# zilliztech/knowhere

Hardware: AMD Instinct MI355X
Metric: QPS at recall@10>=0.95, IVF-PQ 100M x d=128 batch=10k (higher is better)
Workload: dtype f32

## Files before the change

knowhere_amd/csrc/kernels.h:

```cpp
#pragma once

#include <hip/hip_runtime.h>
#include <stdint.h>
#include <algorithm>
#include "sq_codec.h"

namespace knhip {

struct KnItem {
    int32_t list;
    int32_t npair;
    int64_t pair0;
};
struct KnPair {
    int32_t q;
    int32_t slot;
};

__host__ __device__ constexpr int pq_stream_phase(int lane) {
    const int l = lane & 31;
    return l < 4 ? l : l < 12 ? l + 4 : l < 16 ? l - 8 : l < 20 ? l - 16 : l < 28 ? l - 12 : l - 24;
}
constexpr int PQ_STREAM_PHASES = 16;
__host__ __device__ constexpr uint32_t pq_stream_mask(int j) {
// ... 117 lines not shown
    const int64_t* list_sblk_off;
    const int64_t* list_len;
    const int64_t* list_row_off;
    const int64_t* ids;
    const float* precomp_t;
    const float* cb;
    const float* centroids;
    int32_t d;
    int32_t lut_mode;
    const float* queries;
    const float* t2t;
    const float* coarse_dis;
    const KnItem* items;
    const KnPair* pairs;
    const int64_t* nitems_dev;
    const uint8_t* bitset;
    int64_t bitset_nbits;
    float* partial_d;
    int64_t* partial_i;
    float* gthr;
    int32_t nslot;
    int32_t k;
    const int64_t* item_lo;
    const int64_t* item_hi;
    float* dump;
    int64_t dump_stride;
    int32_t dump_by_row;
    const int64_t* dump_pair_col;
    uint32_t* ghist;
    const uint2* gmeta;
    P4Rec* recs4;
    int32_t* q4_ctr;
    const float4* cb_t;
};


struct SqScanArgs {
    const uint4* rows;
    const int64_t* list_blk_off;
    const int64_t* list_len;
    const int64_t* list_row_off;
    const int64_t* ids;
    const float* trained;
    const float* centroids;
    int32_t d;
    int32_t nchunk16;
    int32_t bits;
    const float* queries;
    const float* coarse_dis;
    const KnItem* items;
    const KnPair* pairs;
    const int64_t* nitems_dev;
    const uint8_t* bitset;
    int64_t bitset_nbits;
    float* partial_d;
    int64_t* partial_i;
    float* gthr;
    int32_t nslot;
    int32_t k;
    float* dump;
    int64_t dump_stride;
    const int64_t* dump_pair_col;
    int32_t item_loop;
};

struct MScanArgs {
    const void* rows;
    const float* xnorm;
    float xnorm_max;
    const int64_t* list_blk_off;
    const int64_t* list_len;
    const int64_t* list_row_off;
    const int64_t* ids;
    const float* trained;
    const float* centroids;
    int32_t d;
    int32_t nchunk;
    int32_t nstep;
    int32_t sq_bits;
    int32_t row_type;
    const float* queries;
    const float* qnorm;
    const float* coarse_dis;
    int64_t nq;
    int32_t nslot;
    const KnItem* units;
    const KnPair* pairs;
    const int64_t* nunits_dev;
    const float* gthr;
    float eps_scale;
    const uint8_t* bitset;
    int64_t bitset_nbits;
    int32_t* cand_cnt;
    int64_t* cand;
    uint32_t* eps_max;
    float* cand_pess;
    int32_t cap;
    int32_t* overflow;
    float* dump;
    int64_t dump_stride;
    int32_t sample_cap;
    uint32_t* ghist;
    const uint2* gmeta;
    int32_t k;
    const int32_t* sample_off;
    const void* qh;
    const void* ql;
    const float* qs;
    int32_t unit_loop;
    float* gthr_rw;
    const uint4* pq_codes_r;
    const int64_t* pq_sblk_off_r;
    const float* pq_psum;
    const void* pq_qh;
    const float* pq_qs;
    const float4* pq_cb_t;
    const float* pq_precomp_t;
    const uint8_t* pq_codes;
    int32_t pq_lut_mode;
    P8Rec* pq_recs;
    const uint4* pq_codes_i;
    const void* pq_qi;
    const float* pq_qis;
    P16Rec* pq_recs16;
    int32_t* pq_ctr;
    int32_t pq_prune_mu;
    const void* pq_cb16;
    const void* pq_qh16;
    const float* pq_qd;
    const float* pq_sc;
    const float* pq_psum_s;
    unsigned char* pq_spill;
    int32_t pq_spill_cap;
    int32_t pq_spill_wgs;
    const int2* pq_unit_tiles;
};

int64_t pq_stream16r_blocks(int64_t len);
hipError_t launch_pq_stream16r(const uint8_t* codes, const int64_t* list_row_off, const int64_t* list_len,
                               const int64_t* list_sblk_off, int64_t nlist, uint4* out, hipStream_t s);
hipError_t launch_pq_psum(const uint8_t* codes, const int64_t* list_row_off, const int64_t* list_len,
                          const int64_t* list_sblk_off, int64_t nlist, const float* precomp_t, float* psum,
                          uint32_t* pabs_max_bits, hipStream_t s);
hipError_t launch_pqf_query_table(const float* queries, const float4* cb_m, int d, int64_t nq, bool is_l2, float pabs_max,
                                  void* qh, float* qs, hipStream_t s);
hipError_t launch_pqf_predict(const float* dump, int64_t stride, const int32_t* n_row, const float* gthr, const float* qs,
                              const float* qs2, const int64_t* keys, int nprobe, int64_t nlist, const int64_t* list_len,
                              int64_t nq, int cap, int k, bool is_l2, int32_t* poor, hipStream_t s);
size_t pqf_smem();
hipError_t launch_pq_stream16i(const uint8_t* codes, const int64_t* list_row_off, const int64_t* list_len,
                               const int64_t* list_sblk_off, int64_t nlist, uint4* out, hipStream_t s);
hipError_t launch_pqi_query_table(const float* queries, const float4* cb_m, int d, int64_t nq, bool is_l2, float pabs_max,
                                  void* qi, float* qis, float* qmu, bool stats_done, hipStream_t s);
hipError_t launch_pq_sample(const MScanArgs& a, const int64_t* keys, const float4* cb_m, int64_t nlist, int smin,
                            int scap, float pabs_max, bool is_l2, int32_t* n_row, float* qs, float* qis, float* qmu,
                            hipStream_t s, float* gthr_out = nullptr, uint2* gmeta_out = nullptr, int ksel = 0);
hipError_t launch_pqi(const MScanArgs& a, bool is_l2, int64_t units_bound, hipStream_t s);

constexpr int PD_QT = 128;
size_t pqd_smem();
bool pqd_supports(int M, int d);
hipError_t launch_pqd_index_prep(const float4* cb, const float* centroids, int64_t ncent, void* cb16, float* st,
                                 uint32_t* scratch, const float* psum, int64_t npsum, float* psum_s, hipStream_t s);
hipError_t launch_pqd_query_prep(const float* queries, const float4* cb, const float* cst, int64_t nq, bool is_l2,
                                 float pabs_max, void* qh16, float* qd, hipStream_t s);
hipError_t launch_pqd(const MScanArgs& a, bool is_l2, int64_t units_bound, hipStream_t s);

bool pqf_supports(int M, int d);
hipError_t launch_pqf(const MScanArgs& a, bool is_l2, int64_t units_bound, hipStream_t s);

int flat_scan_qg(int k);
int sq_scan_qg(int k);
hipError_t launch_flat_scan(const FlatScanArgs& a, bool is_l2, bool dense, int64_t grid, hipStream_t s,
                            int qg_override = 0);
hipError_t launch_flat_full(const FlatScanArgs& a, bool is_l2, float* out, const int32_t* q_subset,
                            int64_t nq_subset, const int32_t* row_flags, hipStream_t s);
hipError_t launch_interleave_rows(const float* src, int64_t n, int d, float4* dst, int64_t dst_blk0,
                                  hipStream_t s);
hipError_t launch_rows_narrow_check(const float* x, int64_t n, int d, int row_type, uint16_t* out,
                                    unsigned long long* first_bad, hipStream_t s);
hipError_t launch_rows_widen(const uint16_t* x, int64_t n_values, int row_type, float* out, hipStream_t s);
hipError_t launch_interleave_lists16(const uint16_t* src, const int64_t* list_row_off, const int64_t* list_len,
                                     const int64_t* list_blk_off, int64_t nlist, int d, uint4* dst, hipStream_t s);
hipError_t launch_interleave_lists(const float* src, const int64_t* list_row_off,
                                   const int64_t* list_len, const int64_t* list_blk_off, int64_t nlist,
                                   int d, float4* dst, hipStream_t s);

int pq_scan_supported_m(int M);
int pq_scan_qg(int M);
int64_t pq_skew_blocks(int64_t len, int M);
hipError_t launch_pq_scan(const PqScanArgs& a, bool is_l2, int M, int64_t grid, hipStream_t s);
hipError_t launch_pq_query_table(const float* queries, const float* cb, int d, int M, int64_t nq,
                                 float* t2t, hipStream_t s);
hipError_t launch_pq_precomp_table(const float* centroids, const float* cb, int d, int M,
                                   int64_t nlist, float* pt, hipStream_t s);
hipError_t launch_pq_skew_codes(const uint8_t* codes, const int64_t* list_row_off,
                                const int64_t* list_len, const int64_t* list_sblk_off, int64_t nlist,
                                int M, uint4* out, hipStream_t s);

bool pq_scan_v2_supports(int M, int k);
int64_t pq_stream16_blocks(int64_t len);
hipError_t launch_pq_scan_v2(const PqScanArgs& a, bool is_l2, bool dump, int64_t grid, hipStream_t s);
hipError_t launch_rank0_select(const float* dump, int64_t dump_stride, const int64_t* keys, int nprobe,
                               const int64_t* list_len, const int64_t* list_row_off, const int64_t* ids,
                               int64_t nq, int k, bool is_l2, float* partial_d, int64_t* partial_i, float* gthr,
                               int64_t* tmp_keys, float* tmp_d, uint32_t* ghist, uint2* gmeta, hipStream_t s);
hipError_t launch_pq_stream16(const uint8_t* codes, const int64_t* list_row_off, const int64_t* list_len,
                              const int64_t* list_sblk_off, int64_t nlist, uint4* out, hipStream_t s);

bool pq_scan_q4_supports(int M, int d, int k);
hipError_t launch_pq_scan_q4(const PqScanArgs& a, bool is_l2, int64_t items_bound, hipStream_t s);
hipError_t launch_pq_cb_transpose(const float* cb, int M, int dsub, float4* cb_t, hipStream_t s);

int mscan_queries_per_unit(int kind, bool sample);
size_t mscan_flat_smem(int nstep);
size_t mscan_sq8_smem(int nstep, int bits = 8);
int mscan_finish_pmax(int cap, int k);
int mscan_sample_rows();
hipError_t launch_ms_block_norms(const float4* rows, int64_t total_blk, int nchunk, float* out, float* out_max,
                                 hipStream_t s, int row_type = KN_ROW_FP32);
hipError_t launch_ms_sq8_norms(const uint4* rows, int64_t total_blk, int nchunk16, int d, const float* trained,
                               float* out, float* out_max, hipStream_t s, int bits = 8);
hipError_t launch_ms_units(const int32_t* list_count_v, const int64_t* list_pair_off_v, int64_t nlist, int qt,
                           int64_t* unit_off, int64_t* nunits, KnItem* units, const int64_t* list_len,
                           int64_t code_size, double* unit_bytes, hipStream_t s, int cost_cap = 0,
                           int2* unit_tiles = nullptr);
inline int64_t ms_units_cost_bound(int64_t npairs, int qt, int64_t nlist, int64_t ntotal, int64_t max_len, int cost_cap) {
    const int64_t groups = npairs / qt + std::min<int64_t>(nlist, npairs) + 1;
    if (cost_cap <= 0) {
        return groups;
    }
    const int64_t max_ntile = std::max<int64_t>((max_len + 31) / 32, 1);
    const int64_t by_cost = groups + (2 * max_ntile * (npairs / 32 + groups) + cost_cap - 1) / cost_cap;
    const int64_t by_tiles = npairs / qt * max_ntile + ntotal / 32 + 2 * nlist + 1;
    return std::max<int64_t>(groups, std::min<int64_t>(by_cost, by_tiles));
}
hipError_t launch_mscan_flat(const MScanArgs& a, bool is_l2, int64_t units_bound, hipStream_t s);
int mscan_flat_bf16_qt(int nstep);
size_t mscan_flat_bf16_smem(int nstep);
hipError_t launch_mscan_flat_bf16(const MScanArgs& a, bool is_l2, int64_t units_bound, hipStream_t s);
hipError_t launch_mscan_sq8(const MScanArgs& a, bool is_l2, int64_t units_bound, hipStream_t s);
hipError_t launch_ms_sample_plan(const int64_t* keys, int64_t nq, int nprobe, int64_t nlist, const int64_t* list_len,
                                 int smin, int cap, int32_t* sample_off, int32_t* n_row, hipStream_t s);
hipError_t launch_ms_sq8_query_prep(const float* queries, int64_t nq, int d, int ldq, const float* trained, void* qh,
                                    void* ql, float* qs, hipStream_t s, int bits = 8);
hipError_t launch_ms_tau(const float* sel_d, int64_t nq, int k, bool is_l2, float* gthr, uint2* gmeta, hipStream_t s);
hipError_t launch_mscan_finish(const MScanArgs& a, int kind, bool is_l2, const int64_t* keys, const float* coarse_dis,
                               int nprobe, int k, float* out_d, int64_t* out_i, unsigned long long* counters, int pass,
                               hipStream_t s);
hipError_t launch_ms_flag_pairs(const int32_t* overflow, int want, const int64_t* keys, int64_t nq, int nprobe,
                                int64_t nlist, const int64_t* list_len, int k, KnItem* items, KnPair* pairs,
                                int64_t* nitems, int64_t* empty_mark, hipStream_t s);

hipError_t launch_sq_scan(const SqScanArgs& a, bool is_l2, int64_t grid, hipStream_t s, int qg_override = 0);
hipError_t launch_sq_interleave(const uint8_t* codes, const int64_t* list_row_off,
                                const int64_t* list_len, const int64_t* list_blk_off, int64_t nlist,
                                int64_t code_size, uint4* out, hipStream_t s);

struct WorkTable {
    int32_t* list_count;
    int64_t* list_pair_off;
    int64_t* list_item_off;
    int32_t* list_cursor;
    KnPair* pairs;
    KnItem* items;
    int64_t* nitems;
    double* scan_bytes;
    int64_t* empty_mark;
    int32_t k;
};
hipError_t launch_direct_items(const int64_t* keys, int64_t nq, int nprobe, int64_t nlist, const int64_t* list_len,
                               const WorkTable& wt, hipStream_t s);
hipError_t launch_build_worktable(const int64_t* keys, int64_t nq, int nprobe, int64_t nlist, int qg0, int qg1,
                                  const int64_t* list_len, int64_t code_size, const WorkTable& wt,
                                  hipStream_t s, int rank0_slot = 0, const int32_t* cls = nullptr);
hipError_t launch_fill_f32(float* p, int64_t n, float v, hipStream_t s);

struct RangeArgs {
    const float* dist;
    int64_t ncol;
    const int64_t* seg_col;
    const int64_t* seg_idpos;
    const int64_t* seg_len;
    const int64_t* ids;
    int64_t id_offset;
    const int64_t* order;
    int32_t nprobe;
    float radius;
    const uint8_t* bitset;
    int64_t bitset_nbits;
    const float* radius_q;
    int32_t inclusive;
};
hipError_t launch_tie_detect(const float* d, const int64_t* i, int64_t nq, int k, float* out_d, int64_t* out_i,
                             int32_t* flagged, int32_t* nflag, hipStream_t s);
hipError_t launch_tie_gather(const int32_t* flagged, int nflag, const float* q, int d, const int64_t* keys, const float* cdis,
                             int nprobe, float* q_out, int64_t* keys_out, float* cdis_out, const float* can_d, int k,
                             float* rad_out, hipStream_t s);
hipError_t launch_tie_sort_flags(const int32_t* in, int n, int32_t* out, hipStream_t s);
hipError_t launch_refine_combine(const float* parts, int nsh, int64_t n, float* out, hipStream_t s);
hipError_t launch_tie_resolve(const int32_t* flagged, int nflag, int nsh, const float* can_d, const int64_t* can_i, int k,
                              bool is_l2, const float* arr_d, const int64_t* arr_i, const int64_t* arr_key,
                              const int64_t* arr_n, int64_t arr_n_stride, float* out_d, int64_t* out_i, int32_t* anomalies,
                              hipStream_t s);
struct PqDumpArgs {
    float* dist;
    int64_t ncol;
    const int64_t* pair_col;
    const int64_t* keys;
    const float* coarse_dis;
    int32_t nprobe;
    int64_t nlist;
    const int64_t* list_len;
    const int64_t* list_row_off;
// ... 184 lines not shown
```

knowhere_amd/csrc/knhip_api.hip:

```cpp
#include "knhip_internal.h"

namespace knhip_host {

thread_local std::string g_last_error;

int fail(int code, const std::string& msg) {
    g_last_error = msg;
    return code;
}

int build_coarse_layout(knhip_index* idx) {
    const int nchunk = (idx->d + 3) / 4;
    const int64_t nblk = (idx->nlist + 63) / 64;
    HIP_TRY(idx->centroids_il.alloc((size_t)nblk * nchunk * 64 * sizeof(float4)));
    HIP_TRY(launch_interleave_rows(idx->centroids.as<float>(), idx->nlist, idx->d,
                                   idx->centroids_il.as<float4>(), 0, nullptr));
    HIP_TRY(idx->cnorm.alloc((size_t)idx->nlist * sizeof(float)));
    HIP_TRY(launch_row_norms(idx->centroids.as<float>(), idx->nlist, idx->d, idx->cnorm.as<float>(), nullptr));
    HIP_TRY(idx->centroids_bs.alloc((size_t)idx->nlist * coarse_bf16_slabs(idx->d) * 128));
    HIP_TRY(launch_coarse_bf16_split(idx->centroids.as<float>(), idx->nlist, idx->d, idx->centroids_bs.p, nullptr));
    HIP_TRY(hipDeviceSynchronize());
    std::vector<float> cn((size_t)idx->nlist);
    HIP_TRY(hipMemcpy(cn.data(), idx->cnorm.p, cn.size() * sizeof(float), hipMemcpyDeviceToHost));
    idx->cnorm_max = cn.empty() ? 0.f : *std::max_element(cn.begin(), cn.end());
// ... 255 lines not shown
    idx->h_list_blk_off = blk_off;
    if (kind == KNHIP_IVF_FLAT && idx->row_type != KNHIP_ROWTYPE_FP32) {
        const int nchunk = row_nchunk(idx->d, idx->row_type);
        HIP_TRY(idx->rows.alloc((size_t)total_blk * nchunk * 64 * sizeof(uint4)));
        HIP_TRY(launch_interleave_lists16(reinterpret_cast<const uint16_t*>(d_codes), idx->d_list_row_off.as<int64_t>(),
                                          idx->d_list_len.as<int64_t>(), idx->d_list_blk_off.as<int64_t>(), nlist, idx->d,
                                          idx->rows.as<uint4>(), nullptr));
    } else if (kind == KNHIP_IVF_FLAT) {
        const int nchunk = (idx->d + 3) / 4;
        HIP_TRY(idx->rows.alloc((size_t)total_blk * nchunk * 64 * sizeof(float4)));
        HIP_TRY(launch_interleave_lists(reinterpret_cast<const float*>(d_codes),
                                        idx->d_list_row_off.as<int64_t>(), idx->d_list_len.as<int64_t>(),
                                        idx->d_list_blk_off.as<int64_t>(), nlist, idx->d,
                                        idx->rows.as<float4>(), nullptr));
    } else if (kind == KNHIP_IVF_PQ) {
        const int M = idx->desc.pq_m;
        idx->pq_v2 = (M == 32) && !idx->pq_v1;
        idx->rows.release();
        idx->skew_ready = false;
        if (!idx->pq_v2 && pq_scan_supported_m(M)) {
            if (int rc2 = build_pq_skew(idx)) return rc2;
        }
        if (idx->pq_v2) {
            std::vector<int64_t> off2(nlist + 1, 0);
            for (int64_t l = 0; l < nlist; l++) {
                off2[l + 1] = off2[l] + pq_stream16_blocks(idx->h_list_len[l]);
            }
            if ((rc = upload(idx->d_list_blk_off2, off2.data(), (nlist + 1) * sizeof(int64_t)))) return rc;
            HIP_TRY(idx->rows2.alloc((size_t)off2[nlist] * 64 * sizeof(uint4)));
            HIP_TRY(launch_pq_stream16(d_codes, idx->d_list_row_off.as<int64_t>(), idx->d_list_len.as<int64_t>(),
                                       idx->d_list_blk_off2.as<int64_t>(), nlist, idx->rows2.as<uint4>(), nullptr));
        }
    } else if (kind == KNHIP_IVF_SQ8) {
        const int nchunk16 = sq_nchunk16(idx->d, idx->sq_bits);
        HIP_TRY(idx->rows.alloc((size_t)total_blk * nchunk16 * 64 * sizeof(uint4)));
        HIP_TRY(launch_sq_interleave(d_codes, idx->d_list_row_off.as<int64_t>(),
                                     idx->d_list_len.as<int64_t>(), idx->d_list_blk_off.as<int64_t>(),
                                     nlist, idx->code_size, idx->rows.as<uint4>(), nullptr));
    } else {
        return fail(KNHIP_ERR_INVALID_ARGS, "lists on a brute-force index");
    }
    HIP_TRY(hipDeviceSynchronize());
    if (!keep_aos) {
        idx->codes_aos.release();
    }
    idx->has_data = true;
    return KNHIP_OK;
}

int ensure_aos(const knhip_index* cidx) {
    knhip_index* idx = const_cast<knhip_index*>(cidx);
    if (idx->aos_ready || !idx->has_data || idx->desc.kind == KNHIP_BRUTE_FORCE) {
        return KNHIP_OK;
    }
    HIP_TRY(idx->codes_aos.alloc((size_t)std::max<int64_t>(idx->ntotal, 1) * idx->dev_code_size()));
    HIP_TRY(launch_deinterleave_lists(idx->rows.as<uint4>(), idx->d_list_row_off.as<int64_t>(),
                                      idx->d_list_len.as<int64_t>(), idx->d_list_blk_off.as<int64_t>(), idx->nlist,
                                      idx->dev_code_size(), idx->codes_aos.as<uint8_t>(), nullptr));
    HIP_TRY(hipDeviceSynchronize());
    idx->aos_ready = true;
    return KNHIP_OK;
}

int ensure_mscan_norms(const knhip_index* idx) {
    const int64_t total_blk = idx->total_blk;
    std::lock_guard<std::mutex> lk(idx->mu);
    if (idx->xnorm_ready) {
        return KNHIP_OK;
    }
    HIP_TRY(idx->xnorm.alloc((size_t)std::max<int64_t>(total_blk, 1) * 64 * sizeof(float) + 16));
    float* xn = idx->xnorm.as<float>();
    float* xmax = xn + std::max<int64_t>(total_blk, 1) * 64;
    if (idx->desc.kind == KNHIP_IVF_FLAT) {
        HIP_TRY(launch_ms_block_norms(idx->rows.as<float4>(), total_blk, row_nchunk(idx->d, idx->row_type), xn, xmax, nullptr,
                                      idx->row_type));
        HIP_TRY(hipDeviceSynchronize());
        HIP_TRY(hipMemcpy(&idx->xnorm_max, xmax, sizeof(float), hipMemcpyDeviceToHost));
    } else {
        HIP_TRY(launch_ms_sq8_norms(idx->rows.as<uint4>(), total_blk, sq_nchunk16(idx->d, idx->sq_bits), idx->d,
                                    idx->sq_trained.as<float>(), xn, xmax, nullptr, idx->sq_bits));
        HIP_TRY(hipDeviceSynchronize());
        HIP_TRY(hipMemcpy(&idx->xnorm_max, xmax, sizeof(float), hipMemcpyDeviceToHost));
    }
    idx->xnorm_ready = true;
    return KNHIP_OK;
}

int ensure_psum(const knhip_index* idx) {
    std::lock_guard<std::mutex> lk(idx->mu);
    if (idx->psum_ready) {
        return KNHIP_OK;
    }
    const int64_t nlist = idx->nlist;
    std::vector<int64_t> off(nlist + 1, 0);
    for (int64_t l = 0; l < nlist; l++) {
        off[l + 1] = off[l] + pq_stream16r_blocks(idx->h_list_len[l]);
    }
    HIP_TRY(idx->d_list_blk_off_r.alloc((size_t)(nlist + 1) * sizeof(int64_t)));
    HIP_TRY(hipMemcpy(idx->d_list_blk_off_r.p, off.data(), (size_t)(nlist + 1) * sizeof(int64_t), hipMemcpyHostToDevice));
    idx->pabs_max = 0.f;
    if (idx->is_l2) {
        const size_t npos = (size_t)std::max<int64_t>(off[nlist], 1) * 16;
        HIP_TRY(idx->psum.alloc((npos + 4) * sizeof(float)));
        HIP_TRY(hipMemset(idx->psum.p, 0, (npos + 4) * sizeof(float)));
        uint32_t* bits = reinterpret_cast<uint32_t*>(idx->psum.as<float>() + npos);
        HIP_TRY(launch_pq_psum(idx->codes_aos.as<uint8_t>(), idx->d_list_row_off.as<int64_t>(),
                               idx->d_list_len.as<int64_t>(), idx->d_list_blk_off_r.as<int64_t>(), nlist,
                               idx->precomp_t.as<float>(), idx->psum.as<float>(), bits, nullptr));
        HIP_TRY(hipDeviceSynchronize());
        HIP_TRY(hipMemcpy(&idx->pabs_max, bits, sizeof(float), hipMemcpyDeviceToHost));
    }
    HIP_TRY(hipDeviceSynchronize());
    idx->psum_ready = true;
    return KNHIP_OK;
}

int ensure_pqf(const knhip_index* idx) {
    if (int rc = ensure_psum(idx)) return rc;
    std::lock_guard<std::mutex> lk(idx->mu);
    if (idx->pqf_ready) {
        return KNHIP_OK;
    }
    const int64_t nblk = idx->nlist > 0 ? [&] {
        int64_t t = 0;
        for (int64_t l = 0; l < idx->nlist; l++) t += pq_stream16r_blocks(idx->h_list_len[l]);
        return t;
    }() : 0;
    HIP_TRY(idx->rows_r.alloc((size_t)std::max<int64_t>(nblk, 1) * 64 * sizeof(uint4)));
    HIP_TRY(launch_pq_stream16r(idx->codes_aos.as<uint8_t>(), idx->d_list_row_off.as<int64_t>(),
                                idx->d_list_len.as<int64_t>(), idx->d_list_blk_off_r.as<int64_t>(), idx->nlist,
                                idx->rows_r.as<uint4>(), nullptr));
    HIP_TRY(hipDeviceSynchronize());
    idx->pqf_ready = true;
    return KNHIP_OK;
}

int ensure_pqd(const knhip_index* idx) {
    if (int rc = ensure_psum(idx)) return rc;
    std::lock_guard<std::mutex> lk(idx->mu);
    if (idx->pqd_ready) {
        return KNHIP_OK;
    }
    HIP_TRY(idx->pqd_cb16.alloc((size_t)32 * 256 * 4 * 2));
    HIP_TRY(idx->pqd_st.alloc(16 * sizeof(float)));
    const int64_t npsum = idx->is_l2 ? (int64_t)(idx->psum.bytes / sizeof(float)) - 4 : 0;
    if (npsum > 0) {
        HIP_TRY(idx->psum_s.alloc((size_t)(npsum + 64) * sizeof(float)));
        HIP_TRY(hipMemset(idx->psum_s.p, 0, (size_t)(npsum + 64) * sizeof(float)));
    }
    HIP_TRY(launch_pqd_index_prep(idx->cb.as<float4>(), idx->centroids.as<float>(), idx->nlist * (int64_t)idx->d,
                                  idx->pqd_cb16.p, idx->pqd_st.as<float>(),
                                  reinterpret_cast<uint32_t*>(idx->pqd_st.as<float>() + 8), idx->psum.as<float>(), npsum,
                                  idx->psum_s.as<float>(), nullptr));
    HIP_TRY(hipDeviceSynchronize());
    idx->pqd_ready = true;
    return KNHIP_OK;
}

int ensure_pqi(const knhip_index* idx) {
    if (int rc = ensure_pqf(idx)) return rc;
    std::lock_guard<std::mutex> lk(idx->mu);
    if (idx->pqi_ready) {
        return KNHIP_OK;
    }
    const int64_t nblk = idx->rows_r.bytes / (64 * sizeof(uint4));
    HIP_TRY(idx->rows_i.alloc((size_t)std::max<int64_t>(nblk, 1) * 64 * sizeof(uint4)));
    HIP_TRY(launch_pq_stream16i(idx->codes_aos.as<uint8_t>(), idx->d_list_row_off.as<int64_t>(),
                                idx->d_list_len.as<int64_t>(), idx->d_list_blk_off_r.as<int64_t>(), idx->nlist,
                                idx->rows_i.as<uint4>(), nullptr));
    HIP_TRY(hipDeviceSynchronize());
    idx->pqi_ready = true;
    return KNHIP_OK;
}

Workspace* acquire_ws(const knhip_index* idx, void* stream_key, bool pooled_by_stream) {
    std::lock_guard<std::mutex> lk(idx->mu);
    if (pooled_by_stream) {
        auto& slot = idx->ws_by_stream[stream_key];
        if (!slot) {
            slot.reset(new Workspace());
        }
        return slot.get();
    }
    if (!idx->ws_free.empty()) {
        Workspace* w = idx->ws_free.back().release();
        idx->ws_free.pop_back();
        return w;
    }
    return new Workspace();
}

void release_ws(const knhip_index* idx, Workspace* w) {
    std::lock_guard<std::mutex> lk(idx->mu);
    idx->ws_free.emplace_back(w);
}

int ensure_bf_split(const knhip_index* idx) {
    std::lock_guard<std::mutex> lk(idx->mu);
    if (idx->bf_split_ready) {
        return KNHIP_OK;
    }
    const int64_t nb = idx->ntotal;
    const int nslab = coarse_bf16_slabs(idx->d);
    HIP_TRY(idx->rows_bs.alloc((size_t)std::max<int64_t>(nb, 1) * nslab * 128));
    HIP_TRY(idx->bf_norm.alloc((size_t)std::max<int64_t>(nb, 1) * sizeof(float)));
    HIP_TRY(launch_coarse_bf16_split(idx->codes_aos.as<float>(), nb, idx->d, idx->rows_bs.p, nullptr));
    HIP_TRY(launch_row_norms(idx->codes_aos.as<float>(), nb, idx->d, idx->bf_norm.as<float>(), nullptr));
    HIP_TRY(hipDeviceSynchronize());
    std::vector<float> h((size_t)nb);
    HIP_TRY(hipMemcpy(h.data(), idx->bf_norm.p, h.size() * sizeof(float), hipMemcpyDeviceToHost));
    float mx = 0.f;
    for (float v : h) {
        mx = v > mx ? v : mx;
    }
    idx->bf_norm_max = mx;
    idx->bf_split_ready = true;
    return KNHIP_OK;
}

void note_route(const knhip_index* idx, bool bf_mfma, int pq_form, bool rank0_phase, int64_t items_bound) {
    std::lock_guard<std::mutex> lk(idx->mu);
    idx->last_bf_mfma = bf_mfma ? 1 : 0;
    idx->last_pq_form = pq_form;
    idx->rank0_phase_used = rank0_phase;
    idx->last_items_bound = items_bound;
}

}

extern "C" {

int knhip_device_memory(int32_t device, int64_t* free_bytes, int64_t* total_bytes) {
    int n = 0;
    if (hipGetDeviceCount(&n) != hipSuccess || device < 0 || device >= n) {
        return fail(KNHIP_ERR_INVALID_ARGS, "device_memory: no such device");
    }
    DeviceGuard g(device);
    size_t f = 0, t = 0;
    HIP_TRY(hipMemGetInfo(&f, &t));
    if (free_bytes) *free_bytes = (int64_t)f;
    if (total_bytes) *total_bytes = (int64_t)t;
    return KNHIP_OK;
}

int knhip_abi_version(void) {
    return KNHIP_ABI_VERSION;
}

int knhip_device_count(void) {
    int n = 0;
    if (hipGetDeviceCount(&n) != hipSuccess) {
        return 0;
    }
    return n;
}

const char* knhip_last_error(void) {
    return g_last_error.c_str();
}

int knhip_index_create(const knhip_desc* desc, knhip_index** out) {
    if (!desc || !out) {
        return fail(KNHIP_ERR_INVALID_ARGS, "null argument");
    }
    *out = nullptr;
    if (desc->kind < KNHIP_BRUTE_FORCE || desc->kind > KNHIP_IVF_SQ8) {
        return fail(KNHIP_ERR_INVALID_ARGS, "unknown index kind");
    }
    if (desc->metric != KNHIP_L2 && desc->metric != KNHIP_IP) {
        return fail(KNHIP_ERR_INVALID_ARGS, "metric must be L2 or IP (cosine is normalised IP)");
    }
    if (desc->dim <= 0 || desc->dim > 32768) {
        return fail(KNHIP_ERR_INVALID_ARGS, "dim out of range");
    }
    if (desc->kind != KNHIP_BRUTE_FORCE && (desc->nlist <= 0 || desc->nlist > (1 << 24))) {
        return fail(KNHIP_ERR_INVALID_ARGS, "nlist out of range");
    }
    if (desc->kind == KNHIP_IVF_PQ) {
        if (desc->pq_nbits < 1 || desc->pq_nbits > 8) {
            return fail(KNHIP_ERR_NOT_IMPLEMENTED, "PQ codes of 1 .. 8 bits are supported");
        }
        if (desc->pq_m <= 0 || desc->dim % desc->pq_m != 0) {
            return fail(KNHIP_ERR_INVALID_ARGS, "pq_m must divide dim");
        }
        if (!pq_scan_supported_m(desc->pq_m) && !pq_scan_any_supports(desc->pq_m, desc->dim)) {
            return fail(KNHIP_ERR_NOT_IMPLEMENTED, "pq_m above 128, or sub-vectors of more than 144 dimensions");
        }
    }
    int ndev = knhip_device_count();
    if (ndev <= 0) {
        return fail(KNHIP_ERR_HIP_RUNTIME, "no HIP device visible");
    }
    if (desc->device < 0 || desc->device >= ndev) {
        return fail(KNHIP_ERR_INVALID_ARGS, "device ordinal out of range");
    }
    std::unique_ptr<knhip_index> idx(new knhip_index());
    idx->desc = *desc;
    idx->is_l2 = desc->metric == KNHIP_L2;
    idx->d = desc->dim;
    idx->nlist = desc->kind == KNHIP_BRUTE_FORCE ? 0 : desc->nlist;
    switch (desc->kind) {
        case KNHIP_BRUTE_FORCE:
        case KNHIP_IVF_FLAT:
            idx->code_size = (int64_t)desc->dim * 4;
            break;
        case KNHIP_IVF_PQ:
// ... 997 lines not shown
    }
    return KNHIP_OK;
}

int knhip_index_get_sq(const knhip_index* idx, float* vmin, float* vdiff) {
    if (int rc = check_index(idx)) return rc;
    if (!idx->has_sq || !vmin || !vdiff) {
        return fail(KNHIP_ERR_NOT_TRAINED, "SQ parameters not set");
    }
    DeviceGuard g(idx->desc.device);
    HIP_TRY(hipMemcpy(vmin, idx->sq_trained.p, (size_t)idx->d * sizeof(float), hipMemcpyDeviceToHost));
    HIP_TRY(hipMemcpy(vdiff, idx->sq_trained.as<float>() + idx->d, (size_t)idx->d * sizeof(float), hipMemcpyDeviceToHost));
    return KNHIP_OK;
}

int knhip_index_get_list_sizes(const knhip_index* idx, int64_t* sizes) {
    if (int rc = check_index(idx)) return rc;
    if (idx->desc.kind == KNHIP_BRUTE_FORCE || !sizes) {
        return fail(KNHIP_ERR_INVALID_ARGS, "get_list_sizes: not an IVF index");
    }
    for (int64_t l = 0; l < idx->nlist; l++) {
        sizes[l] = idx->has_data ? idx->h_list_len[l] : 0;
    }
    return KNHIP_OK;
}

int knhip_index_get_lists(const knhip_index* idx, uint8_t* codes, int64_t* ids) {
    if (int rc = check_index(idx)) return rc;
    if (!idx->has_data) {
        return KNHIP_OK;
    }
    DeviceGuard g(idx->desc.device);
    std::lock_guard<std::mutex> add_lk(const_cast<knhip_index*>(idx)->add_mu);
    if (codes) {
        if (int rc = ensure_aos(idx)) return rc;
        const size_t b = idx->desc.kind == KNHIP_BRUTE_FORCE ? (size_t)idx->ntotal * idx->d * sizeof(float)
                                                             : (size_t)idx->ntotal * idx->code_size;
        if (idx->desc.kind == KNHIP_IVF_PQ && idx->desc.pq_nbits != 8) {
            const int nb_pq = idx->desc.pq_nbits, M = idx->desc.pq_m;
            const size_t cs_out = ((size_t)M * nb_pq + 7) / 8;
            std::vector<uint8_t> h(b);
            HIP_TRY(hipMemcpy(h.data(), idx->codes_aos.p, b, hipMemcpyDeviceToHost));
            std::memset(codes, 0, (size_t)idx->ntotal * cs_out);
            for (int64_t i = 0; i < idx->ntotal; i++) {
                uint8_t* dst = codes + (size_t)i * cs_out;
                const uint8_t* src = h.data() + (size_t)i * M;
                for (int m = 0; m < M; m++) {
                    const size_t bit = (size_t)m * nb_pq;
                    const uint32_t v = (uint32_t)src[m] << (bit & 7);
                    dst[bit >> 3] |= (uint8_t)v;
                    if ((bit & 7) + (size_t)nb_pq > 8) {
                        dst[(bit >> 3) + 1] |= (uint8_t)(v >> 8);
                    }
                }
            }
        } else if (idx->row_type != KNHIP_ROWTYPE_FP32) {
            DevBuf wide;
            HIP_TRY(wide.alloc(b));
            HIP_TRY(launch_rows_widen(idx->codes_aos.as<uint16_t>(), idx->ntotal * idx->d, idx->row_type, wide.as<float>(), nullptr));
            HIP_TRY(hipMemcpy(codes, wide.p, b, hipMemcpyDeviceToHost));
        } else {
            HIP_TRY(hipMemcpy(codes, idx->codes_aos.p, b, hipMemcpyDeviceToHost));
        }
    }
    if (ids && idx->desc.kind != KNHIP_BRUTE_FORCE) {
        HIP_TRY(hipMemcpy(ids, idx->ids.p, (size_t)idx->ntotal * sizeof(int64_t), hipMemcpyDeviceToHost));
    }
    return KNHIP_OK;
}

int knhip_index_get_vectors_device(const knhip_index* idx, const float** d_rows) {
    if (int rc = check_index(idx)) return rc;
    if (idx->desc.kind != KNHIP_BRUTE_FORCE || !d_rows) {
        return fail(KNHIP_ERR_INVALID_ARGS, "get_vectors_device: brute-force index only");
    }
    *d_rows = idx->codes_aos.as<float>();
    return KNHIP_OK;
}

int knhip_profile_enable(knhip_index* idx, int on) {
    if (int rc = check_index(idx)) return rc;
    idx->prof = on != 0;
    return KNHIP_OK;
}

static void drain_pending(const knhip_index* idx) {
    std::vector<PendingEvent> p;
    {
        std::lock_guard<std::mutex> lk(idx->mu);
        p.swap(idx->pending);
    }
    for (auto& e : p) {
        float ms = 0.f;
        if (hipEventSynchronize(e.e1) == hipSuccess && hipEventElapsedTime(&ms, e.e0, e.e1) == hipSuccess) {
            idx->times.ms[e.stage] += ms;
            idx->times.launches[e.stage] += 1;
        }
        (void)hipEventDestroy(e.e0);
        (void)hipEventDestroy(e.e1);
    }
}

int knhip_profile_reset(knhip_index* idx) {
    if (int rc = check_index(idx)) return rc;
    DeviceGuard g(idx->desc.device);
    drain_pending(idx);
    std::memset(&idx->times, 0, sizeof(idx->times));
    idx->coarse_flops = 0;
    idx->tie_queries = 0;
    HIP_TRY(hipDeviceSynchronize());
    HIP_TRY(hipMemset(idx->scan_bytes_dev.p, 0, 3 * sizeof(double)));
    HIP_TRY(hipMemset(idx->coarse_fail_dev.p, 0, 8 * sizeof(unsigned long long)));
    return KNHIP_OK;
}

int knhip_profile_get(const knhip_index* idx, knhip_stage_times* out) {
    if (int rc = check_index(idx)) return rc;
    if (!out) {
        return fail(KNHIP_ERR_INVALID_ARGS, "null output");
    }
    DeviceGuard g(idx->desc.device);
    HIP_TRY(hipDeviceSynchronize());
    drain_pending(idx);
    double sb[3] = {0, 0, 0};
    HIP_TRY(hipMemcpy(sb, idx->scan_bytes_dev.p, 3 * sizeof(double), hipMemcpyDeviceToHost));
    *out = idx->times;
    out->scan_bytes = sb[0];
    out->scan_bytes_rank0 = idx->rank0_phase_used ? sb[1] : 0.0;
    out->coarse_flops = idx->coarse_flops;
    out->tie_queries = idx->tie_queries;
    out->scan_items = idx->last_items_bound;
    unsigned long long nf[6] = {0, 0, 0, 0, 0, 0};
    HIP_TRY(hipMemcpy(nf, idx->coarse_fail_dev.p, sizeof(nf), hipMemcpyDeviceToHost));
    out->tie_anomalies = (int64_t)(nf[5] & 0xffffffffull);
    out->coarse_fallback_queries = (int64_t)nf[0];
    out->mscan_queries = (int64_t)nf[1];
    out->mscan_overflow_queries = (int64_t)nf[2];
    out->mscan_candidates = (int64_t)nf[3];
    out->mscan_recomputed = (int64_t)nf[4];
    out->pq_filter_form = idx->desc.kind == KNHIP_BRUTE_FORCE ? (idx->last_bf_mfma ? 10 : 0) : idx->last_pq_form;
    out->mscan_stream_bytes = sb[2];
    return KNHIP_OK;
}

const char* knhip_stage_kernel_name(int stage, int kind) {
    switch (stage) {
        case KNHIP_STAGE_COARSE:
            return "coarse_bf16_kernel (two passes)+coarse_bound_kernel+coarse_rerank_kernel | coarse_gemm_kernel+row_select_thr_kernel";
        case KNHIP_STAGE_GROUP:
            return "wt_*_kernel+ms_unit*_kernel";
        case KNHIP_STAGE_LUT:
            return "pq_query_table_kernel";
        case KNHIP_STAGE_SCAN_RANK0:
            return kind == KNHIP_IVF_PQ ? "pq_sample_kernel | pq_scan_v2_kernel<DUMP>+row_select_kernel"
                                        : "mscan_flat_kernel<DUMP> | mscan_sq8_kernel<DUMP> +row_select_kernel+ms_tau_kernel";
        case KNHIP_STAGE_TABLES:
            return "pqi_query_table_kernel | pqf_query_table_kernel +pqf_predict_kernel";
        case KNHIP_STAGE_SCAN:
            return kind == KNHIP_IVF_PQ    ? "pqi_kernel | pqf_kernel | pq_scan_q4_kernel | pq_scan_kernel | pq_scan_any_kernel"
                   : kind == KNHIP_IVF_SQ8 ? "mscan_sq8_kernel | sq_scan_kernel"
                                           : "mscan_flatb_kernel | mscan_flat_kernel | flat_scan_kernel";
        case KNHIP_STAGE_MERGE:
            return "mscan_finish_kernel | merge_partials_kernel";
        case KNHIP_STAGE_REFINE:
            return "refine_kernel";
        case KNHIP_STAGE_TIES:
            return "tie_detect_kernel+range dump pass+tie_resolve_kernel";
        default:
            return "other";
    }
}

}
```

knowhere_amd/csrc/knhip_api_search.hip:

```cpp
#include "knhip_internal.h"

namespace knhip_host {

template <class A>
static A scan_args(const knhip_index* idx, const Workspace* ws, const Batch& b) {
    A a{};
    a.list_len = idx->d_list_len.as<int64_t>();
    a.list_row_off = idx->d_list_row_off.as<int64_t>();
    a.ids = idx->ids.as<int64_t>();
    a.d = idx->d;
    a.queries = b.q;
    a.bitset = b.bitset;
    a.bitset_nbits = b.nbits;
    a.partial_d = ws->partial_d.as<float>();
    a.partial_i = ws->partial_i.as<int64_t>();
    a.k = b.k;
    return a;
}
template <class A>
static A item_scan_args(const knhip_index* idx, const Workspace* ws, const Batch& b, const WorkTable& wt) {
    A a = scan_args<A>(idx, ws, b);
    a.items = wt.items;
    a.pairs = wt.pairs;
    a.nitems_dev = wt.nitems;
// ... 338 lines not shown
    a.item_hi = wt.nitems;
    if (plan.pq_rank0) {
        const int64_t stride = round_up(std::max<int64_t>(idx->max_list_len, 64), 64);
        HIP_TRY(ws->dump.reserve((size_t)b.nq * stride * sizeof(float)));
        HIP_TRY(ws->sel_keys.reserve((size_t)b.nq * b.k * sizeof(int64_t)));
        HIP_TRY(ws->sel_d.reserve((size_t)b.nq * b.k * sizeof(float)));
        HIP_TRY(ws->ghist.reserve((size_t)b.nq * 64 * sizeof(uint32_t)));
        HIP_TRY(ws->gmeta.reserve((size_t)b.nq * sizeof(uint2)));
        a.dump = ws->dump.as<float>();
        a.dump_stride = stride;
        a.item_lo = nullptr;
        a.item_hi = wt.list_item_off + nlist;
        const int64_t boundA = round_up(b.nq / plan.qg_rank0 + std::min<int64_t>(nlist, b.nq) + 1, 8);
        {
            StageTimer t(idx, s, KNHIP_STAGE_SCAN_RANK0);
            HIP_TRY(launch_pq_scan_v2(a, is_l2, true, boundA, s));
            HIP_TRY(launch_rank0_select(a.dump, stride, b.keys, b.nprobe, idx->d_list_len.as<int64_t>(),
                                        idx->d_list_row_off.as<int64_t>(), idx->ids.as<int64_t>(), b.nq, b.k, is_l2, a.partial_d,
                                        a.partial_i, a.gthr, ws->sel_keys.as<int64_t>(), ws->sel_d.as<float>(),
                                        idx->cand_hist ? ws->ghist.as<uint32_t>() : nullptr, ws->gmeta.as<uint2>(), s));
        }
        if (idx->cand_hist) {
            a.ghist = ws->ghist.as<uint32_t>();
            a.gmeta = ws->gmeta.as<uint2>();
        }
        a.item_lo = wt.list_item_off + nlist;
        a.item_hi = wt.nitems;
    }
    StageTimer t(idx, s, KNHIP_STAGE_SCAN);
    if (plan.pq_q4) {
        if (int rc = pq_q4_bind(idx, ws, plan.items_bound, &a)) return rc;
        HIP_TRY(launch_pq_scan_q4(a, is_l2, plan.items_bound, s));
    } else {
        HIP_TRY(launch_pq_scan_v2(a, is_l2, false, plan.items_bound, s));
    }
    return KNHIP_OK;
}

hipError_t launch_filter(const knhip_index* idx, const SearchPlan& plan, const PqForm& f, const MScanArgs& x, int64_t bound,
                         hipStream_t s) {
    const int kind = idx->desc.kind;
    const bool is_l2 = idx->is_l2;
    return kind == KNHIP_IVF_FLAT ? ((plan.flat_bf16 && x.dump == nullptr) ? launch_mscan_flat_bf16(x, is_l2, bound, s)
                                                                            : launch_mscan_flat(x, is_l2, bound, s))
         : kind == KNHIP_IVF_SQ8  ? launch_mscan_sq8(x, is_l2, bound, s)
         : (f.form == 3 && x.dump == nullptr) ? launch_pqd(x, is_l2, bound, s)
         : (f.form == 2 && x.dump == nullptr) ? launch_pqi(x, is_l2, bound, s)
                                              : launch_pqf(x, is_l2, bound, s);
}

int ms_common_args(const knhip_index* idx, Workspace* ws, const SearchPlan& plan, const Batch& b, const WorkTable& wt,
                   hipStream_t s, MScanArgs& m) {
    const int kind = idx->desc.kind;
    const int64_t nq = b.nq, nlist = idx->nlist;
    if (kind == KNHIP_IVF_PQ) {
        if (int rc = ensure_psum(idx)) return rc;
    } else {
        if (int rc = ensure_mscan_norms(idx)) return rc;
    }
    const int64_t max_units = std::max(plan.ms_units_bound, plan.ms_bound0);
    HIP_TRY(ws->ms_units.reserve((size_t)max_units * sizeof(KnItem)));
    HIP_TRY(ws->ms_unit_off.reserve((size_t)(nlist + 1) * sizeof(int64_t)));
    HIP_TRY(ws->ms_nunits.reserve(sizeof(int64_t) + 2 * sizeof(double)));
    HIP_TRY(ws->ms_cand.reserve((size_t)nq * plan.ms_cap * sizeof(int64_t)));
    HIP_TRY(ws->ms_cand_pess.reserve((size_t)nq * plan.ms_cap * sizeof(float)));
    if (kind == KNHIP_IVF_SQ8) {
        HIP_TRY(ws->ms_eps_max.reserve((size_t)nq * sizeof(uint32_t)));
        HIP_TRY(hipMemsetAsync(ws->ms_eps_max.p, 0, (size_t)nq * sizeof(uint32_t), s));
    }
    HIP_TRY(ws->ms_cand_cnt.reserve((size_t)(2 * nq + 4) * sizeof(int32_t)));
    HIP_TRY(ws->dump.reserve((size_t)nq * mscan_sample_rows() * sizeof(float)));
    HIP_TRY(ws->sel_keys.reserve((size_t)nq * b.k * sizeof(int64_t)));
    HIP_TRY(ws->sel_d.reserve((size_t)nq * b.k * sizeof(float)));
    HIP_TRY(ws->ghist.reserve((size_t)nq * 64 * sizeof(uint32_t)));
    HIP_TRY(ws->gmeta.reserve((size_t)nq * sizeof(uint2)));
    m = MScanArgs{};
    m.rows = idx->rows.p;
    m.xnorm = idx->xnorm.as<float>();
    m.xnorm_max = idx->xnorm_max;
    m.list_blk_off = idx->d_list_blk_off.as<int64_t>();
    m.list_len = idx->d_list_len.as<int64_t>();
    m.list_row_off = idx->d_list_row_off.as<int64_t>();
    m.ids = idx->ids.as<int64_t>();
    m.trained = idx->sq_trained.as<float>();
    m.centroids = idx->centroids.as<float>();
    m.d = idx->d;
    m.nchunk = plan.ms_nchunk;
    m.nstep = plan.ms_nstep;
    m.sq_bits = kind == KNHIP_IVF_SQ8 ? idx->sq_bits : 0;
    m.row_type = idx->row_type;
    m.queries = b.q;
    m.qnorm = ws->qnorm.as<float>();
    m.coarse_dis = b.cdis;
    m.nq = nq;
    m.nslot = b.nprobe;
    m.units = ws->ms_units.as<KnItem>();
    m.pairs = wt.pairs;
    m.nunits_dev = ws->ms_nunits.as<int64_t>();
    m.gthr = ws->gthr.as<float>();
    m.eps_scale = plan.ms_eps_fp32 + (plan.flat_bf16 ? 6.103515625e-5f : 0.f);
    m.bitset = b.bitset;
    m.bitset_nbits = b.nbits;
    m.cand_cnt = ws->ms_cand_cnt.as<int32_t>();
    m.cand = ws->ms_cand.as<int64_t>();
    m.cand_pess = ws->ms_cand_pess.as<float>();
    m.eps_max = kind == KNHIP_IVF_SQ8 ? ws->ms_eps_max.as<uint32_t>() : nullptr;
    m.cap = plan.ms_cap;
    m.overflow = m.cand_cnt + nq;
    m.gthr_rw = ws->gthr.as<float>();
    m.k = b.k;
    if (idx->cand_hist) {
        m.ghist = ws->ghist.as<uint32_t>();
        m.gmeta = ws->gmeta.as<uint2>();
    }
    if (kind == KNHIP_IVF_PQ) {
        HIP_TRY(ws->pq_recs.reserve((size_t)std::max<int64_t>(max_units, plan.npairs) * sizeof(P8Rec)));
        HIP_TRY(ws->pq_ctr.reserve(8 * 16 * sizeof(int32_t)));
        m.list_blk_off = nullptr;
        m.pq_sblk_off_r = idx->d_list_blk_off_r.as<int64_t>();
        m.pq_psum = idx->psum.as<float>();
        m.pq_cb_t = idx->cb_t.as<float4>();
        m.pq_precomp_t = idx->precomp_t.as<float>();
        m.pq_codes = idx->codes_aos.as<uint8_t>();
        m.pq_lut_mode = plan.lut_mode;
        m.pq_recs = ws->pq_recs.as<P8Rec>();
        m.pq_ctr = ws->pq_ctr.as<int32_t>();
    }
    return KNHIP_OK;
}

int ms_fork_group(const knhip_index* idx, Workspace* ws, const SearchPlan& plan, const Batch& b, const EnvSearch& env,
                  const WorkTable& wt, hipStream_t s, SideJoin* sj, WorkTable* wside) {
    *wside = wt;
    if (!plan.wt1_lazy) {
        if (!env.no_side_stream) {
            HIP_TRY(ws->wt[1].reserve(idx->nlist, plan.npairs, plan.items_bound));
            *wside = ws->wt[1].bind(nullptr, wt.empty_mark, wt.k);
        }
        wside->scan_bytes = reinterpret_cast<double*>(ws->ms_nunits.as<int64_t>() + 1);
    }
    if (env.no_side_stream) {
        return KNHIP_OK;
    }
    if (int rc = ensure_side_stream(ws)) return rc;
    HIP_TRY(hipEventRecord(ws->ev_fork, s));
    HIP_TRY(hipStreamWaitEvent(ws->side, ws->ev_fork, 0));
    HIP_TRY(launch_build_worktable(b.keys, b.nq, b.nprobe, idx->nlist, plan.qg, plan.qg, idx->d_list_len.as<int64_t>(),
                                   idx->dev_code_size(), *wside, ws->side, -1));
    HIP_TRY(hipEventRecord(ws->ev_join, ws->side));
    sj->forked = true;
    return KNHIP_OK;
}

int ms_sample_pass(const knhip_index* idx, Workspace* ws, const SearchPlan& plan, const Batch& b, const EnvSearch& env,
                   const WorkTable& wt, hipStream_t s, MScanArgs& m) {
    const int kind = idx->desc.kind, d = idx->d, k = b.k;
    const bool is_l2 = idx->is_l2;
    const int64_t nq = b.nq, nlist = idx->nlist, sample = mscan_sample_rows();
    StageTimer t(idx, s, KNHIP_STAGE_SCAN_RANK0);
    HIP_TRY(hipMemsetAsync(m.cand_cnt, 0, (size_t)(2 * nq + 1) * sizeof(int32_t), s));
    if (kind == KNHIP_IVF_PQ) {
        HIP_TRY(ws->ms_qs.reserve((size_t)nq * 4 * sizeof(float)));
        HIP_TRY(ws->ms_nrow.reserve((size_t)nq * sizeof(int32_t)));
        m.pq_qs = ws->ms_qs.as<float>();
        if (plan.pq_want_i8) {
            HIP_TRY(ws->ms_qi.reserve((size_t)nq * 256 * 32));
            HIP_TRY(ws->ms_qis.reserve(((size_t)nq * 4 + 4) * sizeof(float)));
            HIP_TRY(ws->ms_qmu.reserve((size_t)nq * 32 * sizeof(float)));
        }
    } else if (kind == KNHIP_IVF_FLAT) {
        HIP_TRY(ws->qnorm.reserve((size_t)nq * sizeof(float)));
        m.qnorm = ws->qnorm.as<float>();
        HIP_TRY(launch_row_norms(b.q, nq, d, ws->qnorm.as<float>(), s));
    } else if (!is_l2) {
        const int ldq = plan.ms_nstep * (idx->sq_bits == 8 ? 32 : 64);
        HIP_TRY(ws->ms_qh.reserve((size_t)nq * ldq * 2));
        HIP_TRY(ws->ms_ql.reserve((size_t)nq * ldq * 2));
        HIP_TRY(ws->ms_qs.reserve((size_t)nq * 8 * sizeof(float)));
        HIP_TRY(launch_ms_sq8_query_prep(b.q, nq, d, ldq, idx->sq_trained.as<float>(), ws->ms_qh.p, ws->ms_ql.p,
                                         ws->ms_qs.as<float>(), s, idx->sq_bits));
        m.qh = ws->ms_qh.p;
        m.ql = ws->ms_ql.p;
        m.qs = ws->ms_qs.as<float>();
    }
    HIP_TRY(hipMemsetAsync(ws->ghist.p, 0, (size_t)nq * 64 * sizeof(uint32_t), s));
    MScanArgs ds = m;
    ds.eps_scale = plan.ms_eps_fp32;
    ds.dump = ws->dump.as<float>();
    ds.dump_stride = sample;
    ds.sample_cap = plan.ms_sample_cap;
    ds.ghist = nullptr;
    if (kind == KNHIP_IVF_PQ) {
        int scap = (int)sample;
        if (env.pq_sample_rows > 0) {
            scap = std::max(64, std::min((int)sample, env.pq_sample_rows));
        }
        const bool i8 = plan.pq_want_i8;
        HIP_TRY(launch_pq_sample(ds, b.keys, idx->cb.as<float4>(), nlist, std::max(1024, 8 * k), scap, idx->pabs_max, is_l2,
                                 ws->ms_nrow.as<int32_t>(), ws->ms_qs.as<float>(), i8 ? ws->ms_qis.as<float>() : nullptr,
                                 i8 ? ws->ms_qmu.as<float>() : nullptr, s, ws->gthr.as<float>(), ws->gmeta.as<uint2>(), k));
        return KNHIP_OK;
    }
    HIP_TRY(launch_ms_units(wt.list_count, wt.list_pair_off, nlist, plan.ms_qt0, ws->ms_unit_off.as<int64_t>(),
                            ws->ms_nunits.as<int64_t>(), ws->ms_units.as<KnItem>(), idx->d_list_len.as<int64_t>(), idx->dev_code_size(),
                            nullptr, s));
    ds.sample_off = ws->ms_sample_off.as<int32_t>();
    HIP_TRY(launch_filter(idx, plan, PqForm{}, ds, plan.ms_bound0, s));
    HIP_TRY(launch_row_select_var(ws->dump.as<float>(), sample, b.keys, b.nprobe, idx->d_list_len.as<int64_t>(), nq, k, is_l2,
                                  ws->sel_keys.as<int64_t>(), ws->sel_d.as<float>(), s, sample, ws->ms_nrow.as<int32_t>()));
    HIP_TRY(launch_ms_tau(ws->sel_d.as<float>(), nq, k, is_l2, ws->gthr.as<float>(), ws->gmeta.as<uint2>(), s));
    return KNHIP_OK;
}

int pq_bind_form(const knhip_index* idx, Workspace* ws, const SearchPlan& plan, const Batch& b, const EnvSearch& env, hipStream_t s,
                 MScanArgs& m, PqForm* f) {
    const int64_t nq = b.nq;
    if (f->form == 1) {
        if (int rc = ensure_pqf(idx)) return rc;
        m.pq_codes_r = idx->rows_r.as<uint4>();
        HIP_TRY(ws->ms_qh.reserve((size_t)nq * 256 * 32 * 2));
        HIP_TRY(launch_pqf_query_table(b.q, idx->cb.as<float4>(), idx->d, nq, idx->is_l2, idx->pabs_max, ws->ms_qh.p,
                                       ws->ms_qs.as<float>(), s));
        m.pq_qh = ws->ms_qh.p;
    }
    if (f->form == 2) {
        if (int rc = ensure_pqi(idx)) return rc;
        f->qt = 16;
        HIP_TRY(ws->pq_recs16.reserve((size_t)std::max<int64_t>(std::max(plan.ms_units_bound, plan.ms_bound0), plan.npairs) *
                                      sizeof(P16Rec)));
        m.pq_codes_r = idx->rows_r.as<uint4>();
        m.pq_codes_i = idx->rows_i.as<uint4>();
        m.pq_qi = ws->ms_qi.p;
        m.pq_qis = ws->ms_qis.as<float>();
        m.pq_recs16 = ws->pq_recs16.as<P16Rec>();
    }
    if (f->form == 3) {
        f->qt = PD_QT;
        if (env.pqd_unit_cost > 0) {
            f->pqd_cost = env.pqd_unit_cost;
            f->pqd_bound = round_up(ms_units_cost_bound(plan.npairs, PD_QT, idx->nlist, idx->ntotal, idx->max_list_len,
                                                        f->pqd_cost), 8);
            HIP_TRY(ws->ms_units.reserve((size_t)f->pqd_bound * sizeof(KnItem)));
            HIP_TRY(ws->pqd_tiles.reserve((size_t)f->pqd_bound * sizeof(int2)));
            m.units = ws->ms_units.as<KnItem>();
            m.pq_unit_tiles = ws->pqd_tiles.as<int2>();
        }
        m.pq_cb16 = idx->pqd_cb16.p;
        m.pq_qh16 = ws->ms_qh16.p;
        m.pq_qd = ws->ms_qd.as<float>();
        m.pq_sc = idx->pqd_st.as<float>();
        m.pq_psum_s = idx->psum_s.as<float>();
        m.pq_spill_cap = 4 * 8192;
        if (idx->pqd_spill_cap > 0) {
            m.pq_spill_cap = idx->pqd_spill_cap;
        }
        m.pq_spill_wgs = 512;
        int dev = 0, ncu = 0;
        (void)hipGetDevice(&dev);
        if (hipDeviceGetAttribute(&ncu, hipDeviceAttributeMultiprocessorCount, dev) == hipSuccess && ncu > 0) {
            m.pq_spill_wgs = ncu;
        }
        HIP_TRY(ws->pq_spill.reserve((size_t)m.pq_spill_wgs * m.pq_spill_cap * 80));
        m.pq_spill = static_cast<unsigned char*>(ws->pq_spill.p);
    }
    return KNHIP_OK;
}

int pq_choose_form(const knhip_index* idx, Workspace* ws, const SearchPlan& plan, const Batch& b, const EnvSearch& env,
                   hipStream_t s, MScanArgs& m, PqForm* f) {
    const int64_t nq = b.nq, sample = mscan_sample_rows();
    const int k = b.k, nprobe = b.nprobe;
    const bool is_l2 = idx->is_l2;
    const bool want_dec = pqd_supports(idx->desc.pq_m, idx->d) && (idx->pqf_form == 0 || idx->pqf_form == 3);
    if (plan.pq_want_i8) {
        HIP_TRY(launch_pqi_query_table(b.q, idx->cb.as<float4>(), idx->d, nq, is_l2, idx->pabs_max, ws->ms_qi.p,
                                       ws->ms_qis.as<float>(), ws->ms_qmu.as<float>(), true, s));
    }
    if (want_dec) {
        if (int rc = ensure_pqd(idx)) return rc;
        HIP_TRY(ws->ms_qh16.reserve((size_t)nq * 128 * 2));
        HIP_TRY(ws->ms_qd.reserve((size_t)nq * 4 * sizeof(float)));
        HIP_TRY(launch_pqd_query_prep(b.q, idx->cb.as<float4>(), idx->pqd_st.as<float>(), nq, is_l2, idx->pabs_max,
                                      ws->ms_qh16.p, ws->ms_qd.as<float>(), s));
    }
    const bool want2 = plan.pq_want_i8 || want_dec;
    const int form2 = want_dec ? 3 : 2;
    const float* qs2 = want_dec ? ws->ms_qd.as<float>() : plan.pq_want_i8 ? ws->ms_qis.as<float>() : nullptr;
    auto decide = [&](const int32_t* poor_h, int64_t n) -> int {
        if (want2 && (idx->pqf_form == form2 || (int64_t)poor_h[1] * 4 <= n)) {
            return form2;
        }
        return (int64_t)poor_h[0] * 4 > n ? 0 : 1;
    };
    int form = want2 ? form2 : 1;
    if (idx->pqf_guard) {
        int32_t* poor = ws->ms_cand_cnt.as<int32_t>() + 2 * nq + 1;
        bool predicted = false;
        auto predict = [&]() -> hipError_t {
            if (predicted) {
                return hipSuccess;
            }
            predicted = true;
            return launch_pqf_predict(ws->dump.as<float>(), sample, ws->ms_nrow.as<int32_t>(), ws->gthr.as<float>(),
                                      ws->ms_qs.as<float>(), qs2, b.keys, nprobe, idx->nlist, idx->d_list_len.as<int64_t>(), nq,
                                      plan.ms_cap, k, is_l2, poor, s);
        };
        bool sync_now = true;
        std::unique_lock<std::mutex> lk(idx->mu);
        const bool cached = idx->guard_cache.size() < 64 || idx->guard_cache.count({k, nprobe}) != 0;
        if (cached) {
            knhip_index::GuardEntry& e = idx->guard_cache[{k, nprobe}];
            if (e.pending && hipEventQuery(e.ev) == hipSuccess) {
                e.pending = false;
                e.form = decide(e.h_poor, e.pending_nq);
            }
            e.age++;
            if (e.form > 0 && !env.guard_sync && (e.age & 63) != 0) {
                sync_now = false;
                form = e.form;
                if (!e.pending && (e.age & 3) == 0) {
                    HIP_TRY(predict());
                    if (e.h_poor == nullptr) {
                        HIP_TRY(hipHostMalloc(reinterpret_cast<void**>(&e.h_poor), 2 * sizeof(int32_t)));
                        HIP_TRY(hipEventCreateWithFlags(&e.ev, hipEventDisableTiming));
                    }
                    HIP_TRY(hipMemcpyAsync(e.h_poor, poor, 2 * sizeof(int32_t), hipMemcpyDeviceToHost, s));
                    HIP_TRY(hipEventRecord(e.ev, s));
                    e.pending = true;
                    e.pending_nq = nq;
                }
            }
        }
        lk.unlock();
        if (sync_now) {
            HIP_TRY(predict());
            int32_t h_poor[2] = {0, 0};
            HIP_TRY(hipMemcpyAsync(h_poor, poor, 2 * sizeof(int32_t), hipMemcpyDeviceToHost, s));
            HIP_TRY(hipStreamSynchronize(s));
            form = decide(h_poor, nq);
            if (cached) {
                lk.lock();
                knhip_index::GuardEntry& e = idx->guard_cache[{k, nprobe}];
                if (!e.pending) {
                    e.form = form;
                }
            }
        }
        if (form == 0) {
            return KNHIP_PQF_ABANDONED;
        }
    }
    f->form = form;
    return pq_bind_form(idx, ws, plan, b, env, s, m, f);
}

int ms_group_units(const knhip_index* idx, Workspace* ws, const SearchPlan& plan, const Batch& b, const PqForm& f,
                   const WorkTable& wside, SideJoin* sj, hipStream_t s, MScanArgs& m) {
    const int64_t nlist = idx->nlist;
    StageTimer t(idx, s, KNHIP_STAGE_GROUP);
    if (sj->forked) {
        if (int rc = sj->join()) return rc;
    } else {
        HIP_TRY(launch_build_worktable(b.keys, b.nq, b.nprobe, nlist, plan.qg, plan.qg, idx->d_list_len.as<int64_t>(),
                                       idx->dev_code_size(), wside, s, -1));
    }
    m.pairs = wside.pairs;
    HIP_TRY(launch_ms_units(wside.list_count + nlist, wside.list_pair_off + nlist, nlist, f.qt, ws->ms_unit_off.as<int64_t>(),
                            ws->ms_nunits.as<int64_t>(), ws->ms_units.as<KnItem>(), idx->d_list_len.as<int64_t>(), idx->dev_code_size(),
                            idx->scan_bytes_dev.as<double>() + 2, s, f.pqd_cost, ws->pqd_tiles.as<int2>()));
    return KNHIP_OK;
}

int rows_exact_scan(const knhip_index* idx, Workspace* ws, const Batch& b, const WorkTable& wt, int64_t grid, bool one_pair,
                    hipStream_t s) {
    if (idx->desc.kind == KNHIP_IVF_FLAT) {
        FlatScanArgs a = flat_scan_args(idx, ws, b, wt);
        a.item_loop = one_pair;
        HIP_TRY(launch_flat_scan(a, idx->is_l2, false, grid, s, one_pair));
    } else {
        SqScanArgs a = sq_scan_args(idx, ws, b, wt);
        a.item_loop = one_pair;
        HIP_TRY(launch_sq_scan(a, idx->is_l2, grid, s, one_pair));
    }
    return KNHIP_OK;
}

int exact_one_pair_items(const knhip_index* idx, Workspace* ws, const SearchPlan& plan, const Batch& b, const WorkTable& wt,
                         hipStream_t s) {
    if (idx->desc.kind != KNHIP_IVF_PQ) {
        return rows_exact_scan(idx, ws, b, wt, std::min<int64_t>(plan.npairs, 4096), true, s);
    }
    if (!plan.pq_q4_ok && !idx->skew_ready) {
        if (int rc = build_pq_skew(idx)) return rc;
    }
    PqScanArgs a = pq_scan_args(idx, ws, b, wt);
    a.item_lo = nullptr;
    a.item_hi = wt.nitems;
    if (plan.pq_q4_ok) {
        if (int rc = pq_q4_bind(idx, ws, plan.npairs, &a)) return rc;
        HIP_TRY(launch_pq_scan_q4(a, idx->is_l2, plan.npairs, s));
    } else {
        HIP_TRY(launch_pq_scan(a, idx->is_l2, idx->desc.pq_m, plan.npairs, s));
    }
    return KNHIP_OK;
}

int ms_finish(const knhip_index* idx, Workspace* ws, const SearchPlan& plan, const Batch& b, const PqForm& f, const WorkTable& wt,
              const MScanArgs& m, hipStream_t s) {
    const int kind = idx->desc.kind, k = b.k, nprobe = b.nprobe;
    const bool is_l2 = idx->is_l2;
    const int64_t nq = b.nq, nlist = idx->nlist;
    StageTimer t(idx, s, KNHIP_STAGE_MERGE);
    unsigned long long* counters = idx->coarse_fail_dev.as<unsigned long long>() + 1;
    MScanArgs mf = m;
    if (f.form == 2) {
        mf.pq_qs = m.pq_qis;
        mf.pq_prune_mu = 1;
    }
    if (f.form == 3) {
        mf.pq_qs = m.pq_qd;
    }
    HIP_TRY(launch_mscan_finish(mf, kind, is_l2, b.keys, b.cdis, nprobe, k, b.out_d, b.out_i, counters, 1, s));
    HIP_TRY(launch_ms_flag_pairs(m.overflow, 2, b.keys, nq, nprobe, nlist, idx->d_list_len.as<int64_t>(), k, wt.items, wt.pairs,
                                 wt.nitems, nullptr, s));
    MScanArgs r = m;
    r.pairs = wt.pairs;
    r.units = wt.items;
    r.nunits_dev = wt.nitems;
    r.unit_loop = 1;
    r.pq_unit_tiles = nullptr;
    r.ghist = nullptr;
    r.gmeta = nullptr;
    HIP_TRY(launch_filter(idx, plan, f, r, plan.npairs, s));
    HIP_TRY(launch_mscan_finish(mf, kind, is_l2, b.keys, b.cdis, nprobe, k, b.out_d, b.out_i, counters, 2, s));
    HIP_TRY(launch_ms_flag_pairs(m.overflow, 1, b.keys, nq, nprobe, nlist, idx->d_list_len.as<int64_t>(), k, wt.items, wt.pairs,
                                 wt.nitems, ws->partial_i.as<int64_t>(), s));
    if (int rc = exact_one_pair_items(idx, ws, plan, b, wt, s)) return rc;
    HIP_TRY(launch_merge_partials(ws->partial_d.as<float>(), ws->partial_i.as<int64_t>(), nq, nprobe, k, (int64_t)nprobe * k, k,
                                  is_l2, b.out_d, b.out_i, s, m.overflow));
    return KNHIP_OK;
}

int run_prefilter(const knhip_index* idx, Workspace* ws, const SearchPlan& plan, const Batch& b, const EnvSearch& env,
                  const WorkTable& wt, hipStream_t s, PqForm* f) {
    MScanArgs m;
    if (int rc = ms_common_args(idx, ws, plan, b, wt, s, m)) return rc;
    SideJoin sj{ws, s};
    WorkTable wside;
    if (int rc = ms_fork_group(idx, ws, plan, b, env, wt, s, &sj, &wside)) return rc;
    if (int rc = ms_sample_pass(idx, ws, plan, b, env, wt, s, m)) return rc;
    f->qt = plan.ms_qt;
    {
        StageTimer t(idx, s, KNHIP_STAGE_TABLES);
        if (idx->desc.kind == KNHIP_IVF_PQ) {
            if (int rc = pq_choose_form(idx, ws, plan, b, env, s, m, f)) return rc;
        }
    }
    if (int rc = ms_group_units(idx, ws, plan, b, *f, wside, &sj, s, m)) return rc;
    {
        StageTimer t(idx, s, KNHIP_STAGE_SCAN);
        HIP_TRY(launch_filter(idx, plan, *f, m, std::max(plan.ms_units_bound, f->pqd_bound), s));
    }
    return ms_finish(idx, ws, plan, b, *f, wt, m, s);
}

int ivf_route(const knhip_index* idx, Workspace* ws, const SearchPlan& plan, const Batch& b, const EnvSearch& env, hipStream_t s,
              PqForm* f) {
    const int kind = idx->desc.kind;
    const bool ms = plan.route == Route::Prefilter;
    HIP_TRY(ws->wt[0].reserve(idx->nlist, plan.npairs, ms ? std::max<int64_t>(plan.npairs, plan.items_bound) : plan.items_bound));
    HIP_TRY(ws->partial_d.reserve((size_t)plan.npairs * b.k * sizeof(float)));
    HIP_TRY(ws->partial_i.reserve((size_t)plan.npairs * b.k * sizeof(int64_t)));
    const WorkTable wt = ws->wt[0].bind(idx->scan_bytes_dev.as<double>(), ws->partial_i.as<int64_t>(), b.k);
    if (!plan.wt1_lazy) {
        if (int rc = build_worktable(idx, ws, plan, b, wt, s)) return rc;
    }
    if (kind == KNHIP_IVF_PQ && plan.lut_mode != PQ_LUT_RESIDUAL && !(plan.pq_q4 && !plan.pq_rank0)) {
        if (int rc = pq_lut_stage(idx, ws, b, s)) return rc;
    }
    if (ms) {
        const int rc_ms = run_prefilter(idx, ws, plan, b, env, wt, s, f);
        if (rc_ms != KNHIP_PQF_ABANDONED) {
            return rc_ms;
        }
        if (int rc = build_worktable(idx, ws, plan, b, wt, s)) return rc;
    }
    if (kind == KNHIP_IVF_PQ) {
        if (int rc = pq_exact_scan(idx, ws, plan, b, wt, s)) return rc;
    } else {
        StageTimer t(idx, s, KNHIP_STAGE_SCAN);
        if (int rc = rows_exact_scan(idx, ws, b, wt, plan.items_bound, false, s)) return rc;
    }
    return merge_stage(idx, ws, b, b.nprobe, s);
}

}

int search_batch(const knhip_index* idx, Workspace* ws, const float* d_q, int64_t nq, int k, int nprobe,
                 const uint8_t* d_bitset, int64_t nbits, int64_t* d_out_i, float* d_out_d,
                 hipStream_t s, const int64_t* pre_keys, const float* pre_cdis) {
    HIP_TRY(ws->gthr.reserve((size_t)nq * sizeof(float)));
    HIP_TRY(launch_fill_f32(ws->gthr.as<float>(), nq, idx->is_l2 ? FLT_MAX : -FLT_MAX, s));
    Batch b{d_q, nq, k, nprobe, d_bitset, nbits, d_out_i, d_out_d, pre_keys, pre_cdis};
    if (idx->desc.kind != KNHIP_BRUTE_FORCE && pre_keys == nullptr) {
        HIP_TRY(ws->keys.reserve((size_t)nq * nprobe * sizeof(int64_t)));
        HIP_TRY(ws->cdis.reserve((size_t)nq * nprobe * sizeof(float)));
        StageTimer t(idx, s, KNHIP_STAGE_COARSE);
        if (int rc = coarse_stage(idx, ws, d_q, nq, nprobe, ws->keys.as<int64_t>(), ws->cdis.as<float>(), s)) {
            return rc;
        }
        b.keys = ws->keys.as<int64_t>();
        b.cdis = ws->cdis.as<float>();
    }
    const EnvSearch env = env_search();
    const SearchPlan plan = plan_search(idx, nq, k, nprobe, d_bitset != nullptr, env);
    PqForm form;
    int rc = KNHIP_OK;
    switch (plan.route) {
        case Route::BfMfma:    rc = bf_mfma_batch(idx, ws, b, plan.bf_per, s); break;
        case Route::BfRows:    rc = bf_rows_batch(idx, ws, b, s); break;
        case Route::PqAny:     rc = pq_any_batch(idx, ws, plan, b, s); break;
        case Route::Exact:
        case Route::Prefilter: rc = ivf_route(idx, ws, plan, b, env, s, &form); break;
    }
    note_route(idx, plan.route == Route::BfMfma, form.form, plan.route == Route::Exact && plan.pq_v2 && plan.pq_rank0,
               plan.items_bound);
    return rc;
}

int validate_search(const knhip_index* idx, int64_t nq, int32_t k, int32_t& nprobe) {
    if (nq < 0 || k <= 0) {
        return fail(KNHIP_ERR_INVALID_ARGS, "nq must be >= 0 and k > 0");
    }
    if (k > KNHIP_MAX_K) {
        return fail(KNHIP_ERR_INVALID_ARGS, "k > 16384 is not supported");
    }
    const int kind = idx->desc.kind;
    if (kind == KNHIP_BRUTE_FORCE) {
        if (!idx->has_data) {
            return fail(KNHIP_ERR_EMPTY_INDEX, "brute-force index holds no vectors");
        }
        return KNHIP_OK;
    }
    if (!idx->has_coarse) {
        return fail(KNHIP_ERR_NOT_TRAINED, "coarse centroids not set");
    }
    if (kind == KNHIP_IVF_PQ && !idx->has_pq) {
        return fail(KNHIP_ERR_NOT_TRAINED, "PQ codebooks not set");
    }
    if (kind == KNHIP_IVF_SQ8 && !idx->has_sq) {
        return fail(KNHIP_ERR_NOT_TRAINED, "SQ parameters not set");
    }
    if (!idx->has_data) {
        return fail(KNHIP_ERR_EMPTY_INDEX, "inverted lists not set");
    }
    if (nprobe <= 0) {
        return fail(KNHIP_ERR_INVALID_ARGS, "nprobe must be > 0");
    }
    if (nprobe > idx->nlist) {
        nprobe = (int32_t)idx->nlist;
    }
    if ((size_t)nprobe > row_select_max_k()) {
        return fail(KNHIP_ERR_NOT_IMPLEMENTED, "nprobe > 65536 is not supported");
    }
    return KNHIP_OK;
}

int64_t query_batch(const knhip_index* idx, int64_t nq, int k, int nprobe) {
    double per_q;
    if (idx->desc.kind == KNHIP_BRUTE_FORCE) {
        const int64_t chunk_rows = bf_chunk_rows(idx->ntotal);
        const int64_t nchunks = (idx->ntotal + chunk_rows - 1) / chunk_rows;
        per_q = (double)nchunks * k * 12.0;
    } else {
        per_q = (double)idx->nlist * 4.0 + (double)nprobe * (12.0 + 8.0 + (double)k * 12.0);
        if ((size_t)nprobe > row_select_lds_max_k()) {
            per_q += 16.0 * nprobe;
        }
        if ((idx->desc.kind == KNHIP_IVF_FLAT || idx->desc.kind == KNHIP_IVF_SQ8) && idx->mscan != 0) {
            per_q += 4.0 * mscan_sample_rows() + 8.0 * 32768.0;
        }
        if (idx->desc.kind == KNHIP_IVF_PQ && idx->pqf != 0) {
            per_q += 4.0 * mscan_sample_rows() + 12.0 * 32768.0 + 16384.0 + 8192.0 + (double)nprobe * (256.0 + 96.0);
        }
        if (idx->desc.kind == KNHIP_IVF_PQ) {
            per_q += 256.0 * idx->desc.pq_m * 4.0;
            if (!pq_scan_supported_m(idx->desc.pq_m)) {
                per_q += (double)nprobe * (pq_scan_any_parts(k) - 1) * (double)k * 12.0;
            }
        }
    }
    const double budget = 8.0 * 1024 * 1024 * 1024;
    int64_t qb = (int64_t)(budget / std::max(per_q, 1.0));
    qb = std::max<int64_t>(qb, 8);
    qb = std::min<int64_t>(qb, 65536 * 16);
    return std::min(qb, std::max<int64_t>(nq, 1));
}

}
```

knowhere_amd/csrc/knhip_env.h:

```cpp
#pragma once
#include <algorithm>
#include <cstdlib>
#include <cstring>

namespace knhip_host {

struct EnvLayout {
    bool coarse_given;
    int coarse_gemm;
    size_t aos_keep_bytes;
    bool rank0_select;
    bool cand_hist;
    int pq_q4;
    int mscan;
    bool flat_bf16;
    int mscan_cap;
    int pqd_spill_cap;
    int pqf;
    bool pqf_guard;
    int pqf_form;
    bool pq_v1;
    bool bf_exact;
    int pq_waves;
};

struct EnvSearch {
    int ms_sample_rows;
    int pq_sample_rows;
    bool no_side_stream;
    bool guard_sync;
    bool range_no_waves;
    bool ties_canonical;
    bool ties_trace;
    int pqd_unit_cost;
    size_t largek_round_bytes;
};
constexpr int KNHIP_PQD_UNIT_COST_DEFAULT = 512;

inline bool env_is(const char* v, const char* what) { return v != nullptr && std::strcmp(v, what) == 0; }
inline int env_digit(const char* v, int lo, int hi, int dflt) { return (v && v[0] >= '0' + lo && v[0] <= '0' + hi) ? v[0] - '0' : dflt; }
inline int env_count(const char* v) { return (v && *v) ? std::max(0, std::atoi(v)) : 0; }

inline EnvLayout env_layout() {
    EnvLayout e{};
    const char* c = std::getenv("KNHIP_COARSE");
    e.coarse_given = c != nullptr;
    e.coarse_gemm = env_is(c, "exact") ? 0 : env_is(c, "fp32") ? 1 : 2;
    const char* keep = std::getenv("KNHIP_AOS_KEEP_MB");
    e.aos_keep_bytes = (keep && *keep) ? (size_t)std::max<long long>(0, std::atoll(keep)) << 20 : (size_t)8 << 30;
    const char* r0 = std::getenv("KNHIP_RANK0");
    e.rank0_select = !(r0 && r0[0] == '0');
    const char* h = std::getenv("KNHIP_HIST");
    e.cand_hist = !(h && h[0] == '0');
    e.pq_q4 = env_digit(std::getenv("KNHIP_Q4"), 0, 2, 2);
    e.mscan = env_digit(std::getenv("KNHIP_MSCAN"), 0, 2, 2);
    e.flat_bf16 = !env_is(std::getenv("KNHIP_MSCAN_FLAT"), "fp32");
    e.mscan_cap = env_count(std::getenv("KNHIP_MSCAN_CAP"));
    e.pqd_spill_cap = env_count(std::getenv("KNHIP_PQD_SPILL"));
    const char* pf = std::getenv("KNHIP_PQF");
    e.pqf = (pf && pf[0] == '1') ? 2 : (pf && pf[0] == '0') ? 0 : 1;
    const char* pg = std::getenv("KNHIP_PQF_GUARD");
    e.pqf_guard = !(pg && pg[0] == '0');
    const char* pm = std::getenv("KNHIP_PQF_FORM");
    e.pqf_form = (pm && pm[0] == 'h') ? 1 : (pm && pm[0] == 'i') ? 2 : (pm && pm[0] == 'd') ? 3 : 0;
    const char* v1 = std::getenv("KNHIP_PQ_V1");
    e.pq_v1 = v1 && v1[0] == '1';
    e.bf_exact = env_is(std::getenv("KNHIP_BF"), "exact");
    const char* w = std::getenv("KNHIP_PQ_WAVES");
    e.pq_waves = w ? std::atoi(w) : 8;
    return e;
}

inline long long env_add_slice_rows(int d) {
    const char* v = std::getenv("KNHIP_ADD_SLICE_ROWS");
    if (v && *v && std::atoll(v) > 0) {
        return std::atoll(v);
    }
    return std::max<long long>(1, ((long long)1 << 30) / ((long long)d * 4));
}

inline EnvSearch env_search() {
    EnvSearch e{};
    const char* a = std::getenv("KNHIP_MS_SAMPLE_ROWS");
    e.ms_sample_rows = a ? std::max(1, std::atoi(a)) : 0;
    const char* b = std::getenv("KNHIP_PQ_SAMPLE_ROWS");
    e.pq_sample_rows = b ? std::max(1, std::atoi(b)) : 0;
    e.no_side_stream = std::getenv("KNHIP_NO_SIDE_STREAM") != nullptr;
    e.guard_sync = std::getenv("KNHIP_PQF_GUARD_SYNC") != nullptr;
    e.range_no_waves = std::getenv("KNHIP_RANGE_NO_WAVES") != nullptr;
    const char* t = std::getenv("KNHIP_TIES");
    e.ties_canonical = t && (t[0] == 'c' || t[0] == 'C' || t[0] == '0');
    e.ties_trace = std::getenv("KNHIP_TIES_TRACE") != nullptr;
    const char* uc = std::getenv("KNHIP_PQD_UNIT_COST");
    e.pqd_unit_cost = (uc && *uc) ? std::max(0, std::atoi(uc)) : KNHIP_PQD_UNIT_COST_DEFAULT;
    const char* lk = std::getenv("KNHIP_LARGEK_ROUND_KB");
    e.largek_round_bytes = (lk && *lk) ? (size_t)std::max<long long>(1, std::atoll(lk)) << 10 : (size_t)2 << 30;
    return e;
}

}
```

knowhere_amd/csrc/knhip_internal.h:

```cpp
#pragma once
#include "../../include/knhip.h"
#include "common.h"
#include "kernels.h"
#include "knhip_env.h"

#include <cstdio>
#include <cstdlib>
#include <cstring>
#include <map>
#include <memory>
#include <mutex>
#include <numeric>
#include <random>
#include <string>
#include <vector>

using namespace knhip;

namespace knhip_host {

int fail(int code, const std::string& msg);

#define HIP_TRY(expr)                                                                              \
    do {                                                                                           \
// ... 78 lines not shown
                         empty_mark,               k};
    }
};

struct Workspace {
    DevBuf coarse_full;
    DevBuf keys;
    DevBuf cdis;
    DevBuf t2t;
    DevBuf partial_d;
    DevBuf partial_i;
    DevBuf gthr;
    DevBuf qnorm;
    DevBuf cand_keys;
    DevBuf cand_approx;
    DevBuf fail_flags;
    DevBuf dump;
    DevBuf sel_keys;
    DevBuf sel_d;
    DevBuf rg_seg, rg_cnt, rg_off, rg_tot, rg_out_i, rg_out_d;
    DevBuf cg_gmin, cg_bound, cg_cnt, cg_qs;
    DevBuf rg_state, rg_keys_w, rg_cdis_w;
    DevBuf recs4;
    DevBuf q4_ctr;
    DevBuf ghist;
    DevBuf gmeta;
    WorkTableBufs wt[2];
    DevBuf ms_qi, ms_qis, ms_qmu, pq_recs16;
    DevBuf rs_ovf;
    DevBuf ms_eps_max;
    DevBuf ms_cand_pess;
    DevBuf ms_units, ms_unit_off, ms_nunits, ms_cand, ms_cand_cnt;
    DevBuf ms_sample_off, ms_nrow;
    DevBuf ms_qh, ms_ql, ms_qs;
    DevBuf pq_recs, pq_ctr;
    DevBuf bf_kth;
    DevBuf ms_qh16, ms_qd, pq_spill;
    DevBuf pqd_tiles;
    DevBuf rs_sort;
    DevBuf h_queries, h_bitset, h_out_d, h_out_i, h_ref_d, h_ref_i;
    DevBuf tie_d, tie_i, tie_flag, tie_q, tie_r, tie_keys, tie_cdis;
    DevBuf tie_arr_d, tie_arr_i, tie_arr_n;
    DevBuf lk_plan, lk_scratch;
    std::mutex mu;
    hipStream_t side = nullptr;
    hipEvent_t ev_fork = nullptr, ev_join = nullptr;
    volatile int32_t* h_word = nullptr;
    int32_t word_seq = 0;
    ~Workspace() {
        if (h_word) (void)hipHostFree(const_cast<int32_t*>(h_word));
        if (ev_fork) (void)hipEventDestroy(ev_fork);
        if (ev_join) (void)hipEventDestroy(ev_join);
        if (side) (void)hipStreamDestroy(side);
    }
};

struct SideJoin {
    Workspace* ws;
    hipStream_t s;
    bool forked = false;
    int join() {
        if (forked) {
            forked = false;
            HIP_TRY(hipStreamWaitEvent(s, ws->ev_join, 0));
        }
        return 0;
    }
    ~SideJoin() {
        (void)join();
    }
};

struct PendingEvent {
    int stage;
    hipEvent_t e0, e1;
};

}
using namespace knhip_host;

struct knhip_index {
    knhip_desc desc{};
    bool is_l2 = true;
    int64_t nlist = 0;
    int d = 0;
    bool has_coarse = false;
    DevBuf centroids;
    DevBuf centroids_il;
    DevBuf cnorm;
    DevBuf centroids_bs;
    float cnorm_max = 0.f;
    int coarse_gemm = 2;
    DevBuf coarse_fail_dev;
    bool has_pq = false;
    DevBuf cb;
    DevBuf precomp_t;
    DevBuf cb_t;
    int use_precomp = 0;
    bool has_sq = false;
    DevBuf sq_trained;
    bool has_data = false;
    int64_t ntotal = 0;
    int64_t code_size = 0;
    int sq_bits = 8;
    int row_type = 0;
    int64_t dev_code_size() const { return row_type != 0 ? 2 * (int64_t)d : code_size; }
    int64_t id_offset = 0;
    std::vector<int64_t> h_list_len, h_list_row_off;
    DevBuf d_list_len, d_list_row_off, d_list_blk_off;
    DevBuf ids;
    DevBuf codes_aos;
    mutable bool aos_ready = false;
    std::vector<int64_t> h_list_off;
    DevBuf rows;
    DevBuf rows2;
    DevBuf d_list_blk_off2;
    bool pq_v2 = false;
    mutable bool skew_ready = false;
    int pq_q4 = 2;
    bool rank0_select = true;
    bool cand_hist = true;
    bool pq_v1 = false;
    mutable bool rank0_phase_used = false;
    int64_t max_list_len = 0;
    int ksub = 256;
    int mscan = 2;
    bool flat_bf16 = true;
    int mscan_cap = 0;
    int pqd_spill_cap = 0;
    mutable bool bf_split_ready = false;
    mutable DevBuf rows_bs, bf_norm;
    mutable float bf_norm_max = 0.f;
    bool bf_mfma = true;
    mutable int last_bf_mfma = 0;
    mutable bool xnorm_ready = false;
    mutable DevBuf xnorm;
    mutable float xnorm_max = 0.f;
    int64_t total_blk = 0;
    DevBuf row_scale;
    int cos_mode = 0;
    std::vector<int64_t> h_list_blk_off;
    int pqf = 1;
    bool pqf_guard = true;
    int pqf_form = 0;
    mutable bool psum_ready = false;
    mutable bool pqf_ready = false;
    mutable bool pqi_ready = false;
    mutable bool pqd_ready = false;
    struct GuardEntry {
        int form = -1;
        int32_t* h_poor = nullptr;
        hipEvent_t ev = nullptr;
        bool pending = false;
        int64_t pending_nq = 0;
        int age = 0;
    };
    mutable std::map<std::pair<int, int>, GuardEntry> guard_cache;
    mutable bool idmap_ready = false;
    mutable DevBuf idmap_ids, idmap_col;
    mutable int64_t last_range_ranks = 0;
    mutable int last_pq_form = 0;
    mutable DevBuf rows_i;
    mutable DevBuf rows_r;
    mutable DevBuf d_list_blk_off_r;
    mutable DevBuf psum;
    mutable DevBuf psum_s;
    mutable DevBuf pqd_cb16;
    mutable DevBuf pqd_st;
    mutable float pabs_max = 0.f;
    mutable std::mutex mu;
    std::mutex add_mu;
    mutable std::map<void*, std::unique_ptr<Workspace>> ws_by_stream;
    mutable std::vector<std::unique_ptr<Workspace>> ws_free;
    bool prof = false;
    mutable std::vector<PendingEvent> pending;
    mutable knhip_stage_times times{};
    DevBuf scan_bytes_dev;
    mutable double coarse_flops = 0;
    mutable int64_t tie_queries = 0;
    mutable DevBuf rg_seg_dev;
    mutable int64_t rg_seg_nseg = -1, rg_seg_ncol = 0;
    mutable int64_t last_items_bound = 0;

    int64_t device_bytes() const {
        const DevBuf* all[] = {&centroids, &centroids_il, &centroids_bs, &cb, &precomp_t, &sq_trained, &d_list_len,
                               &d_list_row_off, &d_list_blk_off, &ids, &rows, &rows2, &d_list_blk_off2, &cb_t, &codes_aos,
                               &rows_r, &d_list_blk_off_r, &psum, &rows_i, &idmap_ids, &idmap_col, &psum_s, &pqd_cb16, &pqd_st, &rows_bs, &bf_norm};
        int64_t t = 0;
        for (auto* b : all) {
            t += (int64_t)b->bytes;
        }
        return t;
    }
};

namespace knhip_host {

struct StageTimer {
    const knhip_index* idx;
    hipStream_t s;
    int stage;
    hipEvent_t e0 = nullptr, e1 = nullptr;
    StageTimer(const knhip_index* i, hipStream_t st, int stg) : idx(i), s(st), stage(stg) {
        if (idx->prof) {
            (void)hipEventCreate(&e0);
            (void)hipEventCreate(&e1);
            (void)hipEventRecord(e0, s);
        }
    }
    ~StageTimer() {
        if (idx->prof) {
            (void)hipEventRecord(e1, s);
            std::lock_guard<std::mutex> lk(idx->mu);
            idx->pending.push_back({stage, e0, e1});
        }
    }
};

inline int check_index(const knhip_index* idx) {
    if (!idx) {
        return fail(KNHIP_ERR_INVALID_ARGS, "null index");
    }
    return KNHIP_OK;
}

inline int64_t round_up(int64_t a, int64_t b) {
    return (a + b - 1) / b * b;
}

inline int upload(DevBuf& dst, const void* src, size_t bytes) {
    HIP_TRY(dst.alloc(bytes));
    if (bytes) {
        HIP_TRY(hipMemcpy(dst.p, src, bytes, hipMemcpyHostToDevice));
    }
    return KNHIP_OK;
}

int coarse_stage(const knhip_index* idx, Workspace* ws, const float* d_q, int64_t nq, int nprobe, int64_t* keys, float* cdis,
                 hipStream_t s);
int maybe_build_precomp(knhip_index* idx);
int build_list_layout(knhip_index* idx, const std::vector<int64_t>& list_off, const uint8_t* d_codes, const int64_t* d_ids);
int narrow_rows(const knhip_index* idx, int64_t n, const float* d_x, DevBuf& out, const char* who);
int ensure_aos(const knhip_index* cidx);
Workspace* acquire_ws(const knhip_index* idx, void* stream_key, bool pooled_by_stream);
void release_ws(const knhip_index* idx, Workspace* w);
int search_batch(const knhip_index* idx, Workspace* ws, const float* d_q, int64_t nq, int k, int nprobe, const uint8_t* d_bitset,
                 int64_t nbits, int64_t* d_out_i, float* d_out_d, hipStream_t s, const int64_t* pre_keys = nullptr,
                 const float* pre_cdis = nullptr);
int validate_search(const knhip_index* idx, int64_t nq, int32_t k, int32_t& nprobe);
int64_t query_batch(const knhip_index* idx, int64_t nq, int k, int nprobe);
struct CoarseRows {
    const float* rows;
    const float4* rows_il;
    const void* rows_bs;
    const float* norm;
    float norm_max;
    int64_t n;
};
struct RowsRun {
    float* kth;
    bool have_bound;
    bool queries_ready;
};
int coarse_rows_stage(const knhip_index* idx, Workspace* ws, const CoarseRows& R, const float* d_q, int64_t nq, int nprobe,
                      int64_t* keys, float* cdis, hipStream_t s, RowsRun* run = nullptr);
int build_pq_skew(const knhip_index* cidx);
int ensure_mscan_norms(const knhip_index* idx);
int ensure_psum(const knhip_index* idx);
int ensure_pqf(const knhip_index* idx);
int ensure_pqd(const knhip_index* idx);
int ensure_pqi(const knhip_index* idx);
int ensure_bf_split(const knhip_index* idx);
void note_route(const knhip_index* idx, bool bf_mfma, int pq_form, bool rank0_phase, int64_t items_bound);
struct Batch {
    const float* q;
    int64_t nq;
    int k, nprobe;
    const uint8_t* bitset;
    int64_t nbits;
    int64_t* out_i;
    float* out_d;
    const int64_t* keys;
    const float* cdis;
};
FlatScanArgs flat_scan_args(const knhip_index* idx, const Workspace* ws, const Batch& b, const WorkTable& wt);
SqScanArgs sq_scan_args(const knhip_index* idx, const Workspace* ws, const Batch& b, const WorkTable& wt);
PqScanArgs pq_scan_args(const knhip_index* idx, const Workspace* ws, const Batch& b, const WorkTable& wt);
PqAnyArgs pq_any_args(const knhip_index* idx, const Workspace* ws, const Batch& b);
inline int pq_lut_mode(const knhip_index* x) { return !x->is_l2 ? PQ_LUT_IP : (x->use_precomp ? PQ_LUT_PRECOMP : PQ_LUT_RESIDUAL); }
inline int64_t bf_chunk_rows(int64_t nb) { return std::max<int64_t>(1024, round_up((nb + 511) / 512, 64)); }
int search_batch_ties(const knhip_index* idx, Workspace* ws, const float* d_q, int64_t nq, int k, int nprobe,
                      const uint8_t* d_bitset, int64_t nbits, int64_t* d_out_i, float* d_out_d, hipStream_t s,
                      const int64_t* pre_keys, const float* pre_cdis);
int add_vectors_common(knhip_index* idx, int64_t n, const float* d_x, const int64_t* d_ids, int64_t id_offset);
}

struct knhip_rows {
    int device = 0, d = 0, row_type = KNHIP_ROWS_FP16;
    int64_t n = 0;
    bool trained = false;
    DevBuf codes;
    DevBuf sq;
    std::mutex mu;
    bool ranged() const { return row_type == KNHIP_ROWS_SQ8 || row_type == KNHIP_ROWS_SQ6 || row_type == KNHIP_ROWS_SQ4U; }
    int nrange() const { return row_type == KNHIP_ROWS_SQ4U ? 1 : d; }
    int64_t code_size() const {
// ... 9 lines not shown
```

knowhere_amd/csrc/ms_common.h:

```cpp
#pragma once
#include "common.h"
#include "kernels.h"

namespace knhip {

template <bool IS_L2>
__device__ __forceinline__ void ms_emit(const MScanArgs& a, int32_t q, int32_t slot, int64_t row_off, int64_t pos,
                                        float pess) {
    if (a.bitset != nullptr && bitset_filtered(a.bitset, a.bitset_nbits, a.ids[row_off + pos])) {
        return;
    }
    const int n = atomicAdd(a.cand_cnt + q, 1);
    if (n < a.cap) {
        a.cand[(int64_t)q * a.cap + n] = ((int64_t)slot << 32) | (int64_t)(uint32_t)pos;
        if (a.cand_pess != nullptr) {
            a.cand_pess[(int64_t)q * a.cap + n] = pess;
        }
    } else {
        a.overflow[q] = 1;
        a.overflow[a.nq] = 1;
    }
    if (a.ghist != nullptr) {
        const uint2 mt = a.gmeta[q];
        if (mt.y != KN_HIST_OFF) {
            atomicAdd(a.ghist + (int64_t)q * KN_HIST_BINS + hist_bin(dist_key<IS_L2>(pess), mt.x, mt.y), 1u);
        }
    }
}

struct MsHist {
    bool on;
    uint2 mt;
    uint32_t cum;
};

__device__ __forceinline__ void ms_hist_load(const MScanArgs& a, int32_t q, MsHist& h) {
    h.on = a.ghist != nullptr && q >= 0;
    if (h.on) {
        h.mt = a.gmeta[q];
        h.cum = __hip_atomic_load(a.ghist + (int64_t)q * KN_HIST_BINS + lane_id(), __ATOMIC_RELAXED,
                                  __HIP_MEMORY_SCOPE_AGENT);
    }
}

template <bool IS_L2>
__device__ __forceinline__ float ms_hist_eval(const MsHist& h, int k) {
    float bound = worst_dist<IS_L2>();
    if (!h.on) {
        return bound;
    }
    const uint2 mt = h.mt;
    if (mt.y == KN_HIST_OFF) {
        return bound;
    }
    const int lane = lane_id();
    uint32_t cum = h.cum;
#pragma unroll
    for (int dlt = 1; dlt < KN_WAVE; dlt <<= 1) {
        const uint32_t up = __shfl_up(cum, dlt, KN_WAVE);
        cum += lane >= dlt ? up : 0u;
    }
    const unsigned long long reach = __ballot(cum >= (uint32_t)k);
    const int b = reach ? __ffsll((long long)reach) - 1 : KN_HIST_BINS;
    if (b < KN_HIST_BINS - 1) {
        const unsigned long long edge = (unsigned long long)mt.x + (((unsigned long long)b + 1ull) << mt.y) - 1ull;
        if (edge < 0xffffffffull) {
            const float e = dist_key_inv<IS_L2>((uint32_t)edge);
            if (e == e && fabsf(e) < FLT_MAX) {
                bound = e;
            }
        }
    }
    return bound;
}

template <bool IS_L2>
__device__ __forceinline__ float ms_hist_bound(const MScanArgs& a, int32_t q, int k) {
    MsHist h;
    ms_hist_load(a, q, h);
    return ms_hist_eval<IS_L2>(h, k);
}

template <bool IS_L2>
__device__ __forceinline__ float ms_hist_bound_lane(const MScanArgs& a, int32_t q, int k) {
    float bound = worst_dist<IS_L2>();
    if (a.ghist == nullptr || q < 0) {
        return bound;
    }
    const uint2 mt = a.gmeta[q];
    if (mt.y == KN_HIST_OFF) {
        return bound;
    }
    const unsigned long long* hp = reinterpret_cast<const unsigned long long*>(a.ghist + (int64_t)q * KN_HIST_BINS);
    unsigned long long w[KN_HIST_BINS / 2];
#pragma unroll
    for (int i = 0; i < KN_HIST_BINS / 2; i++) {
        w[i] = __hip_atomic_load(hp + i, __ATOMIC_RELAXED, __HIP_MEMORY_SCOPE_AGENT);
    }
    uint32_t cum = 0;
    int b = KN_HIST_BINS;
#pragma unroll
    for (int i = 0; i < KN_HIST_BINS / 2; i++) {
        cum += (uint32_t)w[i];
        b = (b == KN_HIST_BINS && cum >= (uint32_t)k) ? 2 * i : b;
        cum += (uint32_t)(w[i] >> 32);
        b = (b == KN_HIST_BINS && cum >= (uint32_t)k) ? 2 * i + 1 : b;
    }
    if (b < KN_HIST_BINS - 1) {
        const unsigned long long edge = (unsigned long long)mt.x + (((unsigned long long)b + 1ull) << mt.y) - 1ull;
        if (edge < 0xffffffffull) {
            const float e = dist_key_inv<IS_L2>((uint32_t)edge);
            if (e == e && fabsf(e) < FLT_MAX) {
                bound = e;
            }
        }
    }
    return bound;
}

__device__ __forceinline__ unsigned long long ms_valid_rows(const MScanArgs& a, int64_t b, int64_t len, int64_t row_off) {
    const int64_t row = b * 64 + lane_id();
    bool v = row < len;
    if (v && a.bitset != nullptr) {
        v = !bitset_filtered(a.bitset, a.bitset_nbits, a.ids[row_off + row]);
    }
    return __ballot(v);
}

}
```

knowhere_amd/csrc/pq_decode.hip:

```cpp
#include "common.h"
#include "kernels.h"
#include "ms_common.h"

#include <algorithm>
#include <cmath>
#include <cstdio>
#include <type_traits>

namespace knhip {

#ifndef PD_EXP
#define PD_EXP 0
#endif
constexpr int PD_M = 32;
constexpr int PD_KSUB = 256;
constexpr int PD_D = 128;
constexpr int PD_WAVES = 4;
constexpr int PD_THREADS = PD_WAVES * KN_WAVE;
constexpr int PD_CB_BYTES = PD_M * PD_KSUB * 8;
constexpr int PD_RING = 8;
constexpr int PD_REC_BYTES = 80;
constexpr int PD_REC_CAP = 176;
constexpr int PD_FLAT_CAP = 256;
constexpr int PD_PA_BYTES = PD_QT * 16;
constexpr int PD_W_PA = 0;
constexpr int PD_W_REC = PD_W_PA + 2 * PD_PA_BYTES;
constexpr int PD_W_FLAT = PD_W_REC + PD_REC_CAP * PD_REC_BYTES;
constexpr int PD_W_PCNT = PD_W_FLAT + PD_FLAT_CAP * 16;
constexpr int PD_W_CTL = PD_W_PCNT + 2 * PD_QT * 4;
constexpr int PD_W_BYTES = PD_W_CTL + 64;
constexpr int PD_OFF_W = PD_CB_BYTES;
constexpr int PD_SMEM = PD_OFF_W + PD_WAVES * PD_W_BYTES;
static_assert(PD_SMEM <= 160 * 1024, "LDS of one workgroup");
constexpr float PD_U = 5.9604645e-8f;
constexpr float PD_UH = 4.8828125e-4f;
constexpr float PD_A = 6.103515625e-5f;

#ifdef KNHIP_PHASE_TIMERS
#define PD_T(i)                                                         \
    do {                                                                \
        const unsigned long long t_ = __builtin_amdgcn_s_memtime();     \
        tacc[i] += t_ - tlast;                                          \
        tlast = t_;                                                     \
    } while (0)
#define PD_COUNT(i, n) tacc[i] += (unsigned long long)(n)
#define PD_TARG , unsigned long long (&tacc)[8], unsigned long long& tlast
#define PD_TPASS , tacc, tlast
__device__ unsigned long long g_pd_prof[4 * 8 + 8];
#else
#define PD_T(i)
#define PD_COUNT(i, n)
#define PD_TARG
#define PD_TPASS
#endif

typedef _Float16 pd_h8 __attribute__((ext_vector_type(8)));
typedef float pd_f16 __attribute__((ext_vector_type(16)));
typedef uint32_t pd_u4 __attribute__((ext_vector_type(4)));
typedef __amdgpu_buffer_rsrc_t pd_rsrc;

size_t pqd_smem() { return PD_SMEM; }

bool pqd_supports(int M, int d) { return M == PD_M && d == PD_D; }

__host__ __device__ inline float pqd_scale_for(float amax) {
    if (!(amax > 0.f) || !(amax < INFINITY)) {
        return 1.0f;
    }
    int e;
    frexpf(amax, &e);
    int s = 15 - e;
    s = s < -60 ? -60 : (s > 60 ? 60 : s);
    return ldexpf(1.0f, s);
}

__global__ __launch_bounds__(PD_KSUB) void pqd_codebook_kernel(const float4* __restrict__ cb, const uint32_t* __restrict__ cmax_bits,
                                                               _Float16* __restrict__ cb16, float* __restrict__ st) {
    __shared__ float s_red[PD_KSUB];
    __shared__ float s_bc[2];
    const int c = threadIdx.x;
    float amax = 0.f;
    for (int m = 0; m < PD_M; m++) {
        const float4 e = cb[m * PD_KSUB + c];
        amax = fmaxf(amax, fmaxf(fmaxf(fabsf(e.x), fabsf(e.y)), fmaxf(fabsf(e.z), fabsf(e.w))));
    }
    s_red[c] = amax;
    __syncthreads();
    if (c == 0) {
        float v = 0.f;
        for (int i = 0; i < PD_KSUB; i++) {
            v = fmaxf(v, s_red[i]);
        }
        s_bc[0] = v;
    }
    __syncthreads();
    const float ymax = s_bc[0];
    const float sc = pqd_scale_for(ymax);
    float ysum = 0.f;
    for (int m = 0; m < PD_M; m++) {
        const float4 e = cb[m * PD_KSUB + c];
        _Float16* o = cb16 + ((size_t)m * PD_KSUB + c) * 4;
        o[0] = (_Float16)(e.x * sc);
        o[1] = (_Float16)(e.y * sc);
        o[2] = (_Float16)(e.z * sc);
        o[3] = (_Float16)(e.w * sc);
        __syncthreads();
        s_red[c] = fabsf(e.x) + fabsf(e.y) + fabsf(e.z) + fabsf(e.w);
        __syncthreads();
        if (c == 0) {
            float v = 0.f;
            for (int i = 0; i < PD_KSUB; i++) {
                v = fmaxf(v, s_red[i]);
            }
            ysum += v;
        }
    }
    if (c == 0) {
        const float cmax = __uint_as_float(*cmax_bits);
        const float sq = pqd_scale_for(4.0f * (cmax + ymax));
        st[0] = sc;
        st[1] = 1.0f / sc;
        st[2] = ymax;
        st[3] = ysum * 1.0001f;
        st[4] = sq;
        st[5] = 1.0f / sq;
        st[6] = sq * sc;
        st[7] = 1.0f / (sq * sc);
    }
}

__global__ __launch_bounds__(256) void pqd_absmax_kernel(const float* __restrict__ x, int64_t n, uint32_t* __restrict__ out) {
    float m = 0.f;
    for (int64_t i = (int64_t)blockIdx.x * blockDim.x + threadIdx.x; i < n; i += (int64_t)gridDim.x * blockDim.x) {
        const float v = fabsf(x[i]);
        m = v < INFINITY ? fmaxf(m, v) : m;
    }
#pragma unroll
    for (int dlt = KN_WAVE / 2; dlt > 0; dlt >>= 1) {
        m = fmaxf(m, __shfl_xor(m, dlt, KN_WAVE));
    }
    if (lane_id() == 0 && m > 0.f) {
        atomicMax(out, __float_as_uint(m));
    }
}

__global__ __launch_bounds__(256) void pqd_scale_psum_kernel(const float* __restrict__ psum, int64_t n, const float* __restrict__ st,
                                                             float* __restrict__ psum_s) {
    const float f = -0.5f * st[6];
    for (int64_t i = (int64_t)blockIdx.x * blockDim.x + threadIdx.x; i < n; i += (int64_t)gridDim.x * blockDim.x) {
        psum_s[i] = psum[i] * f;
    }
}

hipError_t launch_pqd_index_prep(const float4* cb, const float* centroids, int64_t ncent, void* cb16, float* st,
                                 uint32_t* scratch, const float* psum, int64_t npsum, float* psum_s, hipStream_t s) {
    hipError_t e = hipMemsetAsync(scratch, 0, sizeof(uint32_t), s);
    if (e != hipSuccess) {
        return e;
    }
    if (ncent > 0) {
        const unsigned grid = (unsigned)std::min<int64_t>((ncent + 255) / 256, 1024);
        hipLaunchKernelGGL(pqd_absmax_kernel, dim3(grid), dim3(256), 0, s, centroids, ncent, scratch);
    }
    hipLaunchKernelGGL(pqd_codebook_kernel, dim3(1), dim3(PD_KSUB), 0, s, cb, scratch, static_cast<_Float16*>(cb16), st);
    if (npsum > 0 && psum != nullptr) {
        const unsigned grid = (unsigned)std::min<int64_t>((npsum + 255) / 256, 65535);
        hipLaunchKernelGGL(pqd_scale_psum_kernel, dim3(grid), dim3(256), 0, s, psum, npsum, st, psum_s);
    }
    return hipGetLastError();
}

template <bool IS_L2>
__global__ __launch_bounds__(PD_KSUB) void pqd_query_prep_kernel(const float* __restrict__ queries, const float4* __restrict__ cb,
                                                                 const float* __restrict__ cst, float pabs_max,
                                                                 _Float16* __restrict__ qh16, float* __restrict__ qd) {
    __shared__ float s_q[PD_D];
    __shared__ uint32_t s_max[PD_M];
    const int64_t q = blockIdx.x;
    const int c = threadIdx.x;
    if (c < PD_D) {
        s_q[c] = queries[q * PD_D + c];
    }
    if (c < PD_M) {
        s_max[c] = 0u;
    }
    __syncthreads();
    const float inv_y = cst[1], ysum = cst[3], sc_q = cst[4], inv_q = cst[5], inv_sc = cst[7];
    if (c < PD_D) {
        qh16[q * PD_D + c] = (_Float16)(s_q[c] * sc_q);
    }
    for (int m = 0; m < PD_M; m++) {
        const float4 e = cb[m * PD_KSUB + c];
        float v = fabsf(s_q[4 * m]) * fabsf(e.x) + fabsf(s_q[4 * m + 1]) * fabsf(e.y) + fabsf(s_q[4 * m + 2]) * fabsf(e.z) +
                  fabsf(s_q[4 * m + 3]) * fabsf(e.w);
#pragma unroll
        for (int dlt = KN_WAVE / 2; dlt > 0; dlt >>= 1) {
            v = fmaxf(v, __shfl_xor(v, dlt, KN_WAVE));
        }
        if (lane_id() == 0) {
            atomicMax(&s_max[m], __float_as_uint(v));
        }
    }
    __syncthreads();
    if (c == 0) {
        float B = 0.f, q1 = 0.f;
        bool fits = true;
        for (int m = 0; m < PD_M; m++) {
            B += __uint_as_float(s_max[m]);
        }
        for (int i = 0; i < PD_D; i++) {
            q1 += fabsf(s_q[i]);
            fits = fits && fabsf(s_q[i]) * sc_q < 65504.0f;
        }
        B *= 1.0001f;
        q1 *= 1.0001f;
        float eps = INFINITY;
        if (fits && B < INFINITY) {
            const float F = IS_L2 ? 2.0f : 1.0f;
            const float e_prod = (2.0f * PD_UH + PD_UH * PD_UH) * B;
            const float e_sub = PD_A * (1.0f + PD_UH) * (ysum * inv_q + q1 * inv_y) + 128.0f * PD_A * PD_A * inv_sc;
            const float e_acc = 136.0f * PD_U * ((1.0f + 3.0f * PD_UH) * B + 0.5f * pabs_max);
            eps = (F * (e_prod + e_sub + e_acc) + 128.0f * PD_U * (pabs_max + F * B)) * 1.001f;
#if defined(PD_EXP) && (PD_EXP & 32)
            eps *= 16.0f;
#endif
#if defined(PD_EXP) && (PD_EXP & 64)
            eps *= 0.25f;
#endif
        }
        qd[q * 4 + 0] = q1;
        qd[q * 4 + 1] = B;
        qd[q * 4 + 2] = eps;
        qd[q * 4 + 3] = 2.0f * B;
    }
}

hipError_t launch_pqd_query_prep(const float* queries, const float4* cb, const float* cst, int64_t nq, bool is_l2,
                                 float pabs_max, void* qh16, float* qd, hipStream_t s) {
    if (nq <= 0) {
        return hipSuccess;
    }
    if (is_l2) {
        hipLaunchKernelGGL(pqd_query_prep_kernel<true>, dim3((unsigned)nq), dim3(PD_KSUB), 0, s, queries, cb, cst, pabs_max,
                           static_cast<_Float16*>(qh16), qd);
    } else {
        hipLaunchKernelGGL(pqd_query_prep_kernel<false>, dim3((unsigned)nq), dim3(PD_KSUB), 0, s, queries, cb, cst, 0.f,
                           static_cast<_Float16*>(qh16), qd);
    }
    return hipGetLastError();
}

__device__ __forceinline__ float pd_max3(float a, float b, float c) { return fmaxf(fmaxf(a, b), c); }

__device__ __forceinline__ float pd_max16(const pd_f16& v) {
    const float a = pd_max3(v[0], v[1], v[2]), b = pd_max3(v[3], v[4], v[5]), c = pd_max3(v[6], v[7], v[8]);
    const float d = pd_max3(v[9], v[10], v[11]), e = pd_max3(v[12], v[13], v[14]);
    return fmaxf(pd_max3(a, b, c), pd_max3(d, e, v[15]));
}

typedef int pd_i4 __attribute__((ext_vector_type(4)));
#if defined(__HIP_DEVICE_COMPILE__) && !defined(PD_NO_ASM)
#define PD_RING_CLOBBER "a216", "a217", "a218", "a219", "a220", "a221", "a222", "a223", "a224", "a225", "a226", "a227", "a228", "a229", "a230", "a231", "a232", "a233", "a234", "a235", "a236", "a237", "a238", "a239", "a240", "a241", "a242", "a243", "a244", "a245", "a246", "a247", "a248", "a249", "a250", "a251", "a252", "a253", "a254", "a255", "memory"
struct PdRing {};
template <int I, bool WITH_P>
__device__ __forceinline__ void pd_ring_load(PdRing&, pd_i4 rc, int voff_c, int soff_c, pd_i4 rp, int voff_p, int soff_p) {
    static_assert(I >= 0 && I < PD_RING, "eight slots: codes a[216 + 4 I : 219 + 4 I], start value a[248 + I]");
#define PD_LD(WREG, PREG)                                                                                                    \
    if (WITH_P) {                                                                                                            \
        asm volatile("s_nop 4\n\tbuffer_load_dwordx4 " WREG ", %0, %1, %2 offen\n\tbuffer_load_dword " PREG ", %3, %4, %5 offen" \
                     :                                                                                                       \
                     : "v"(voff_c), "s"(rc), "s"(soff_c), "v"(voff_p), "s"(rp), "s"(soff_p)                                  \
                     : PD_RING_CLOBBER);                                                                                     \
    } else {                                                                                                                 \
        asm volatile("s_nop 4\n\tbuffer_load_dwordx4 " WREG ", %0, %1, %2 offen" : : "v"(voff_c), "s"(rc), "s"(soff_c) : PD_RING_CLOBBER); \
    }
    if (I == 0) {
        PD_LD("a[216:219]", "a248")
    } else if (I == 1) {
        PD_LD("a[220:223]", "a249")
    } else if (I == 2) {
        PD_LD("a[224:227]", "a250")
    } else if (I == 3) {
        PD_LD("a[228:231]", "a251")
    } else if (I == 4) {
        PD_LD("a[232:235]", "a252")
    } else if (I == 5) {
        PD_LD("a[236:239]", "a253")
    } else if (I == 6) {
        PD_LD("a[240:243]", "a254")
    } else {
        PD_LD("a[244:247]", "a255")
    }
#undef PD_LD
}
template <int I, int N, bool WITH_P>
__device__ __forceinline__ void pd_ring_take(PdRing&, pd_u4& w, float& p) {
    uint32_t w0, w1, w2, w3;
    float pp = 0.f;
#define PD_TK(W0, W1, W2, W3, PREG)                                                                                          \
    if (WITH_P) {                                                                                                            \
        asm volatile("s_waitcnt vmcnt(%5)\n\tv_accvgpr_read_b32 %0, " W0 "\n\tv_accvgpr_read_b32 %1, " W1                   \
                     "\n\tv_accvgpr_read_b32 %2, " W2 "\n\tv_accvgpr_read_b32 %3, " W3 "\n\tv_accvgpr_read_b32 %4, " PREG "\n\ts_nop 7" \
                     : "=v"(w0), "=v"(w1), "=v"(w2), "=v"(w3), "=v"(pp)                                                      \
                     : "n"(N)                                                                                                \
                     : PD_RING_CLOBBER);                                                                                     \
    } else {                                                                                                                 \
        asm volatile("s_waitcnt vmcnt(%4)\n\tv_accvgpr_read_b32 %0, " W0 "\n\tv_accvgpr_read_b32 %1, " W1                   \
                     "\n\tv_accvgpr_read_b32 %2, " W2 "\n\tv_accvgpr_read_b32 %3, " W3 "\n\ts_nop 7"                          \
                     : "=v"(w0), "=v"(w1), "=v"(w2), "=v"(w3)                                                                \
                     : "n"(N)                                                                                                \
                     : PD_RING_CLOBBER);                                                                                     \
    }
    if (I == 0) {
        PD_TK("a216", "a217", "a218", "a219", "a248")
    } else if (I == 1) {
        PD_TK("a220", "a221", "a222", "a223", "a249")
    } else if (I == 2) {
        PD_TK("a224", "a225", "a226", "a227", "a250")
    } else if (I == 3) {
        PD_TK("a228", "a229", "a230", "a231", "a251")
    } else if (I == 4) {
        PD_TK("a232", "a233", "a234", "a235", "a252")
    } else if (I == 5) {
        PD_TK("a236", "a237", "a238", "a239", "a253")
    } else if (I == 6) {
        PD_TK("a240", "a241", "a242", "a243", "a254")
    } else {
        PD_TK("a244", "a245", "a246", "a247", "a255")
    }
#undef PD_TK
    w[0] = w0;
    w[1] = w1;
    w[2] = w2;
    w[3] = w3;
    p = pp;
}
__device__ __forceinline__ void pd_ring_drain(PdRing&) { asm volatile("s_waitcnt vmcnt(0)" : : : PD_RING_CLOBBER); }
#else
struct PdRing {
    pd_u4 w[PD_RING];
    float p[PD_RING];
};
template <int I, bool WITH_P>
__device__ __forceinline__ void pd_ring_load(PdRing& r, pd_i4 rc, int voff_c, int soff_c, pd_i4 rp, int voff_p, int soff_p) {
    const pd_rsrc dc = __builtin_amdgcn_make_buffer_rsrc(
            reinterpret_cast<void*>(((uint64_t)(uint32_t)rc[1] << 32) | (uint32_t)rc[0]), 0, rc[2], rc[3]);
    r.w[I] = __builtin_amdgcn_raw_buffer_load_b128(dc, voff_c, soff_c, 0);
    r.p[I] = 0.f;
    if (WITH_P) {
        const pd_rsrc dp = __builtin_amdgcn_make_buffer_rsrc(
                reinterpret_cast<void*>(((uint64_t)(uint32_t)rp[1] << 32) | (uint32_t)rp[0]), 0, rp[2], rp[3]);
        r.p[I] = __builtin_bit_cast(float, __builtin_amdgcn_raw_buffer_load_b32(dp, voff_p, soff_p, 0));
    }
}
template <int I, int N, bool WITH_P>
__device__ __forceinline__ void pd_ring_take(PdRing& r, pd_u4& w, float& p) {
    w = r.w[I];
    p = r.p[I];
}
__device__ __forceinline__ void pd_ring_drain(PdRing&) {}
#endif

__device__ __forceinline__ void pd_wave_sync() {
#if defined(__HIP_DEVICE_COMPILE__) && !defined(PD_NO_ASM)
    asm volatile("s_waitcnt lgkmcnt(0)" : : : "memory");
#else
    (void)__ballot(1);
#endif
}

struct PdUnit {
    int64_t len;
    int64_t row_off;
    int64_t ps_off;
    int ntile;
    uint32_t pos0;
};

template <bool IS_L2, int NTQ>
__device__ __forceinline__ int pqd_scan(const MScanArgs& a, unsigned char* smem, unsigned char* wb, const unsigned char* pa,
                                        int wslot, pd_h8 (&B)[4][8], const PdUnit& un PD_TARG) {
    const int lane = lane_id();
    const int lr = lane & 31, hi = lane >> 5;
    const float* sT = reinterpret_cast<const float*>(pa);
    const int32_t* sPq = reinterpret_cast<const int32_t*>(pa + 2 * PD_QT * 4);
    int32_t* ctl = reinterpret_cast<int32_t*>(wb + PD_W_CTL);
// ... 431 lines not shown
                case 2: nrec = pqd_scan<IS_L2, 2>(a, smem, wb, pa, wslot, B, un PD_TPASS); break;
                case 3: nrec = pqd_scan<IS_L2, 3>(a, smem, wb, pa, wslot, B, un PD_TPASS); break;
                default: nrec = pqd_scan<IS_L2, 4>(a, smem, wb, pa, wslot, B, un PD_TPASS); break;
            }
        }
        PD_T(2);
        PairConst cn;
        pair_request(pn, cn);
        pd_wave_sync();
        PD_T(4);
        uint4* flat = reinterpret_cast<uint4*>(wb + PD_W_FLAT);
        auto sort_out = [&](const uint32_t (&rw)[PD_REC_BYTES / 4]) {
            const uint32_t pair = rw[0], row0 = rw[1];
            const float thq = sT[pair];
            uint32_t hm = 0;
#pragma unroll
            for (int r = 0; r < 16; r++) {
                const uint32_t pos = row0 + (uint32_t)((r & 3) + 8 * (r >> 2));
                hm |= (__uint_as_float(rw[4 + r]) >= thq && (int64_t)pos < un.len) ? (1u << r) : 0u;
            }
            while (hm != 0u) {
                const int r = __ffs((int)hm) - 1;
                hm &= hm - 1u;
                uint32_t xb = rw[4];
#pragma unroll
                for (int r2 = 1; r2 < 16; r2++) {
                    xb = r == r2 ? rw[4 + r2] : xb;
                }
                const uint32_t pos = row0 + (uint32_t)((r & 3) + 8 * (r >> 2));
                if (a.bitset != nullptr && bitset_filtered(a.bitset, a.bitset_nbits, a.ids[un.row_off + (int64_t)pos])) {
                    continue;
                }
                const int at = atomicAdd(&ctl[1], 1);
                if (at < PD_FLAT_CAP) {
                    const int rank = atomicAdd(&pcnt[pair], 1);
                    flat[at] = make_uint4(pair, un.pos0 + pos, xb, (uint32_t)rank);
                } else {
                    const float xs = __uint_as_float(xb) * inv_sc, c = sC[pair];
                    ms_emit<IS_L2>(a, sPq[pair], sPs[pair], un.row_off - un.pos0, (int64_t)(un.pos0 + pos),
                                   IS_L2 ? c - 2.0f * xs : c + xs);
                }
            }
        };
        if (nrec > 0) {
            const int n_own = min(nrec, PD_REC_CAP), n_gl = min(ctl[2], a.pq_spill_cap / PD_WAVES);
            for (int i = lane; i < n_own; i += KN_WAVE) {
                uint32_t rw[PD_REC_BYTES / 4];
                const unsigned char* rp = wb + PD_W_REC + i * PD_REC_BYTES;
#pragma unroll
                for (int j = 0; j < PD_REC_BYTES / 16; j++) {
                    const uint4 q4 = reinterpret_cast<const uint4*>(rp)[j];
                    rw[4 * j] = q4.x;
                    rw[4 * j + 1] = q4.y;
                    rw[4 * j + 2] = q4.z;
                    rw[4 * j + 3] = q4.w;
                }
                sort_out(rw);
            }
            const uint32_t* gl = reinterpret_cast<const uint32_t*>(a.pq_spill) +
                                 (int64_t)wslot * (a.pq_spill_cap / PD_WAVES) * (PD_REC_BYTES / 4);
            for (int i = lane; i < n_gl; i += KN_WAVE) {
                uint32_t rw[PD_REC_BYTES / 4];
#pragma unroll
                for (int j = 0; j < PD_REC_BYTES / 4; j++) {
                    rw[j] = __hip_atomic_load(gl + (int64_t)i * (PD_REC_BYTES / 4) + j, __ATOMIC_RELAXED, __HIP_MEMORY_SCOPE_AGENT);
                }
                sort_out(rw);
            }
        }
        pair_write(pn, cn, par ^ 1);
        PD_T(3);
        pd_wave_sync();
#ifdef KNHIP_PHASE_TIMERS
        if (lane == 0) {
            atomicMax(&g_pd_prof[33], (unsigned long long)ctl[2]);
            atomicMax(&g_pd_prof[34], (unsigned long long)ctl[1]);
            atomicAdd(&g_pd_prof[35], (unsigned long long)nrec);
            atomicAdd(&g_pd_prof[36], (unsigned long long)ctl[1]);
            atomicAdd(&g_pd_prof[37], (unsigned long long)(ctl[2] > 0));
        }
#endif
        if (nxt >= 0) {
            load_queries(par ^ 1, (a.units[nxt].npair + 31) >> 5);
        }
        pn = pair_of(nn);
        const int nflat = min(ctl[1], PD_FLAT_CAP);
        if (nflat > 0) {
            static_assert(PD_FLAT_CAP == 4 * KN_WAVE, "four rows per lane");
            uint4 fe[4];
            uint2 mt[4];
#pragma unroll
            for (int b = 0; b < 4; b++) {
                const int i = lane + KN_WAVE * b;
                fe[b] = make_uint4(0u, 0u, 0u, 0u);
                mt[b] = make_uint2(0u, KN_HIST_OFF);
                if (i < nflat) {
                    fe[b] = flat[i];
                    if (a.ghist != nullptr) {
                        mt[b] = a.gmeta[sPq[fe[b].x]];
                    }
                }
            }
#pragma unroll
            for (int h = 0; h < 2; h++) {
                const int j = lane + 64 * h;
                const int c = pcnt[j];
                if (c > 0) {
                    const int32_t q = sPq[j];
                    const int base = atomicAdd(a.cand_cnt + q, c);
                    pbase[j] = base;
                    if (base + c > a.cap) {
                        a.overflow[q] = 1;
                        a.overflow[a.nq] = 1;
                    }
                }
            }
            pd_wave_sync();
#pragma unroll
            for (int b = 0; b < 4; b++) {
                const int i = lane + KN_WAVE * b;
                if (i < nflat) {
                    const uint4 h = fe[b];
                    const int32_t q = sPq[h.x];
                    const float x = __uint_as_float(h.z) * inv_sc, c = sC[h.x];
                    const float pess = IS_L2 ? c - 2.0f * x : c + x;
                    const int n = pbase[h.x] + (int)h.w;
                    if (n < a.cap) {
                        a.cand[(int64_t)q * a.cap + n] = ((int64_t)sPs[h.x] << 32) | (int64_t)h.y;
                        if (a.cand_pess != nullptr) {
                            a.cand_pess[(int64_t)q * a.cap + n] = pess;
                        }
                    }
                    if (mt[b].y != KN_HIST_OFF) {
                        atomicAdd(a.ghist + (int64_t)q * KN_HIST_BINS + hist_bin(dist_key<IS_L2>(pess), mt[b].x, mt[b].y), 1u);
                    }
                }
            }
        }
        cur = nxt;
        nxt = nn;
        par ^= 1;
        pd_wave_sync();
        PD_T(5);
    }
#ifdef KNHIP_PHASE_TIMERS
    if (lane == 0) {
        for (int i = 0; i < 8; i++) {
            atomicAdd(&g_pd_prof[wave * 8 + i], tacc[i]);
        }
    }
#endif
}

hipError_t launch_pqd(const MScanArgs& a, bool is_l2, int64_t units_bound, hipStream_t s) {
    if (units_bound <= 0) {
        return hipSuccess;
    }
    if (a.dump != nullptr || a.pq_spill == nullptr || a.pq_spill_cap <= 0 || a.pq_cb16 == nullptr || a.pq_qh16 == nullptr || a.pq_qd == nullptr || a.pq_sc == nullptr ||
        a.pq_codes == nullptr || a.pq_ctr == nullptr || (is_l2 && (a.pq_psum_s == nullptr || a.pq_sblk_off_r == nullptr))) {
        return hipErrorInvalidValue;
    }
    int dev = 0, ncu = 0;
    (void)hipGetDevice(&dev);
    (void)hipDeviceGetAttribute(&ncu, hipDeviceAttributeMultiprocessorCount, dev);
    if (ncu <= 0) {
        ncu = 256;
    }
    auto kern = a.unit_loop ? (is_l2 ? pqd_kernel<true, true> : pqd_kernel<false, true>)
                            : (is_l2 ? pqd_kernel<true, false> : pqd_kernel<false, false>);
    hipError_t e = hipFuncSetAttribute(reinterpret_cast<const void*>(kern), hipFuncAttributeMaxDynamicSharedMemorySize,
                                       (int)PD_SMEM);
    if (e != hipSuccess) {
        return e;
    }
    if (!a.unit_loop) {
        e = hipMemsetAsync(a.pq_ctr, 0, 8 * 16 * sizeof(int32_t), s);
        if (e != hipSuccess) {
            return e;
        }
    }
    const int64_t grid = std::min<int64_t>(std::min<int64_t>((units_bound + PD_WAVES - 1) / PD_WAVES, ncu), a.pq_spill_wgs);
#ifdef KNHIP_PHASE_TIMERS
    static unsigned long long zero[40] = {0};
    (void)hipMemcpyToSymbol(HIP_SYMBOL(g_pd_prof), zero, sizeof(zero));
#endif
    hipLaunchKernelGGL(kern, dim3((unsigned)grid), dim3(PD_THREADS), PD_SMEM, s, a);
#ifdef KNHIP_PHASE_TIMERS
    (void)hipStreamSynchronize(s);
    unsigned long long h[40];
    (void)hipMemcpyFromSymbol(h, HIP_SYMBOL(g_pd_prof), sizeof(h));
    {
        int64_t nu = -1;
        (void)hipMemcpy(&nu, a.nunits_dev, sizeof(nu), hipMemcpyDeviceToHost);
        fprintf(stderr, "[pqd timers] ring mismatches %llu\n", h[39]);
        fprintf(stderr, "[pqd timers] launch unit_loop=%d units=%lld | max global %llu max flat %llu | parked lanes %llu "
                        "passing rows %llu | units with global records %llu\n", (int)a.unit_loop, (long long)nu, h[33], h[34],
                h[35], h[36], h[37]);
    }
    if (!a.unit_loop) {
        fprintf(stderr, "[pqd timers] ticks per workgroup (grid %lld): wave | prologue  operands  tiles  flush-A  end-barrier  flush-B+barriers | "
                        "tiles  slow entries\n", (long long)grid);
        for (int w = 0; w < 4; w++) {
            fprintf(stderr, "[pqd timers]   %d |", w);
            for (int i = 0; i < 6; i++) fprintf(stderr, " %10.0f", (double)h[w * 8 + i] / (double)grid);
            fprintf(stderr, " | %8.0f %8.0f\n", (double)h[w * 8 + 6] / (double)grid, (double)h[w * 8 + 7] / (double)grid);
        }
    }
#endif
    return hipGetLastError();
}

}
```

knowhere_amd/csrc/pq_filter.hip:

```cpp
#include "common.h"
#include "kernels.h"
#include "ms_common.h"

#include <algorithm>
#include <cstddef>
#include <cstdio>
#include <cstdlib>

namespace knhip {

constexpr int PF_KSUB = 256;
constexpr int PF_M = 32;
constexpr int PF_DSUB = 4;
constexpr int PF_Q = 8;
constexpr int PF_WAVES = 16;
constexpr int PF_THREADS = PF_WAVES * KN_WAVE;
constexpr int PF_LUT_BYTES = PF_KSUB * PF_M * PF_Q * 2;
constexpr int PF_CTL_BYTES = 1536;
constexpr int PF_SAMPLE = 8192;
constexpr int PF_STAGE_CAP = 1792;
constexpr int PF_STAGE_BYTES = PF_STAGE_CAP * 16 + 16;
constexpr float PF_U = 5.9604645e-8f;
constexpr float PF_UH = 4.8828125e-4f;

// ... 839 lines not shown
    for (int m = 0; m < PF_M; m++) {
        const bool fin = fabsf(hi[m]) < INFINITY;
        lo[m] = fin ? hi[m] : -INFINITY;
        hi[m] = fin ? hi[m] : INFINITY;
    }
    const float rh = pf_reduce32(hi, [](float x, float y) { return fmaxf(x, y); });
    const float rl = pf_reduce32(lo, [](float x, float y) { return fminf(x, y); });
    if ((lane_id() & 1) == 0) {
        smax[(lane_id() >> 1) & 31][wave] = rh;
        smin[(lane_id() >> 1) & 31][wave] = rl;
    }
    __syncthreads();
    if (c < PF_M) {
        float h = smax[c][0], l = smin[c][0];
        for (int w = 1; w < PF_KSUB / KN_WAVE; w++) {
            h = fmaxf(h, smax[c][w]);
            l = fminf(l, smin[c][w]);
        }
        const float mu = 0.5f * h + 0.5f * l;
        s_mu[c] = mu;
        s_a[c] = fmaxf(fabsf(h), fabsf(l));
        s_r[c] = h - l;
        qmu[q * PF_M + c] = mu;
    }
    __syncthreads();
    if (c == 0) {
        float A = 0.f, R = 0.f, musum = 0.f;
        for (int m = 0; m < PF_M; m++) {
            musum += s_mu[m];
            A += s_a[m];
            R = fmaxf(R, s_r[m]);
        }
        qis[q * 4 + 0] = R;
        qis[q * 4 + 1] = musum;
        qis[q * 4 + 2] = INFINITY;
        qis[q * 4 + 3] = A;
        if (R > 0.f && R < INFINITY) {
            atomicMax(gl, __float_as_uint(R));
        }
    }
}

template <bool IS_L2>
__global__ __launch_bounds__(PF_KSUB) void pqi_query_table_kernel(const float* __restrict__ queries,
                                                                  const float4* __restrict__ cb_m, int d, float pabs_max,
                                                                  int64_t nq, const float* __restrict__ qmu,
                                                                  uint32_t* __restrict__ qi, float* __restrict__ qis) {
    __shared__ float sq[PF_M * PF_DSUB];
    __shared__ float smu[PF_M];
    __shared__ float s_inv;
    const int64_t q = blockIdx.x;
    const int c = threadIdx.x;
    if (c < PF_M * PF_DSUB) {
        sq[c] = queries[q * d + c];
    }
    if (c < PF_M) {
        smu[c] = qmu[q * PF_M + c];
    }
    if (c == 0) {
        const float s0 = pqi_base_step(__uint_as_float(reinterpret_cast<const uint32_t*>(qis)[nq * 4]));
        const float inv0 = 1.0f / s0;
        if (q == 0) {
            qis[nq * 4 + 1] = s0;
            qis[nq * 4 + 2] = inv0;
        }
        const float R = qis[q * 4 + 0], musum = qis[q * 4 + 1], A = qis[q * 4 + 3];
        float step = s0, eps = INFINITY;
        if (A < INFINITY && R < INFINITY && pabs_max * inv0 < PI_INT_LIM) {
            const float w = fminf(fmaxf(ceilf((R / 254.0f) * inv0), 1.0f), 127.0f);
            step = w * s0;
            eps = 16.4f * step + 128.0f * PF_U * (pabs_max + A) + 64.0f * PF_U * fabsf(musum);
        }
        s_inv = 1.0f / step;
        qis[q * 4 + 0] = step;
        qis[q * 4 + 2] = eps;
    }
    __syncthreads();
    float v[PF_M];
    pq_table_values<IS_L2>(sq, cb_m, c, v);
    const float inv = s_inv;
    uint32_t* out = qi + q * (PF_KSUB * PF_M / 4);
#pragma unroll
    for (int l16 = 0; l16 < 16; l16++) {
        float x0 = rintf((v[l16] - smu[l16]) * inv), x1 = rintf((v[l16 + 16] - smu[l16 + 16]) * inv);
        x0 = fminf(fmaxf(x0, -127.0f), 127.0f);
        x1 = fminf(fmaxf(x1, -127.0f), 127.0f);
        x0 = (x0 == x0) ? x0 : 0.f;
        x1 = (x1 == x1) ? x1 : 0.f;
        const uint32_t pair = ((uint32_t)(int)x0 & 0xffu) | (((uint32_t)(int)x1 & 0xffu) << 8);
        const uint32_t other = (uint32_t)__shfl_xor((int)pair, 1, KN_WAVE);
        if ((c & 1) == 0) {
            out[((c >> 2) * 16 + l16) * 2 + ((c >> 1) & 1)] = pair | (other << 16);
        }
    }
}

hipError_t launch_pqi_query_table(const float* queries, const float4* cb_m, int d, int64_t nq, bool is_l2, float pabs_max,
                                  void* qi, float* qis, float* qmu, bool stats_done, hipStream_t s) {
    if (nq <= 0) {
        return hipSuccess;
    }
    uint32_t* gl = reinterpret_cast<uint32_t*>(qis + nq * 4);
    if (!stats_done) {
        hipError_t e = hipMemsetAsync(qis + nq * 4, 0, 4 * sizeof(float), s);
        if (e != hipSuccess) {
            return e;
        }
        if (is_l2) {
            hipLaunchKernelGGL(pqi_query_stats_kernel<true>, dim3((unsigned)nq), dim3(PF_KSUB), 0, s, queries, cb_m, d,
                               qmu, qis, gl);
        } else {
            hipLaunchKernelGGL(pqi_query_stats_kernel<false>, dim3((unsigned)nq), dim3(PF_KSUB), 0, s, queries, cb_m, d,
                               qmu, qis, gl);
        }
    }
    if (is_l2) {
        hipLaunchKernelGGL(pqi_query_table_kernel<true>, dim3((unsigned)nq), dim3(PF_KSUB), 0, s, queries, cb_m, d,
                           pabs_max, nq, qmu, static_cast<uint32_t*>(qi), qis);
    } else {
        hipLaunchKernelGGL(pqi_query_table_kernel<false>, dim3((unsigned)nq), dim3(PF_KSUB), 0, s, queries, cb_m, d,
                           pabs_max, nq, qmu, static_cast<uint32_t*>(qi), qis);
    }
    return hipGetLastError();
}

constexpr int PS_THREADS = 512;
constexpr int PS_WAVES = PS_THREADS / KN_WAVE;
constexpr int PS_CAND = 1024;
constexpr int PS_ROWS = 2;
template <int NV>
__device__ __forceinline__ uint32_t ps_wave_select(const uint32_t (&v)[NV], int r, uint32_t l, uint32_t h) {
    while (l < h) {
        const uint32_t mid = l + ((h - l) >> 1);
        int cnt = 0;
#pragma unroll
        for (int u = 0; u < NV; u++) {
            cnt += __popcll(__ballot(v[u] <= mid));
        }
        if (cnt >= r) {
            h = mid;
        } else {
            l = mid + 1;
        }
    }
    return l;
}
template <bool IS_L2>
__global__ __launch_bounds__(PS_THREADS) __attribute__((amdgpu_waves_per_eu(8, 8))) void pq_sample_kernel(MScanArgs a, const int64_t* __restrict__ keys,
                                                            const float4* __restrict__ cb_m, int64_t nlist, int smin,
                                                            int scap, float pabs_max, int32_t* __restrict__ n_row,
                                                            float* __restrict__ qs, float* __restrict__ qis,
                                                            float* __restrict__ qmu, uint32_t* __restrict__ gl,
                                                            float* __restrict__ gthr_out, uint2* __restrict__ gmeta_out,
                                                            int ksel) {
    __shared__ float lut[PF_M * PF_KSUB];
    __shared__ float sq[PF_M * PF_DSUB];
    __shared__ float s_mu[PF_M], s_a[PF_M], s_r[PF_M];
    __shared__ float s_A;
    const int64_t q = blockIdx.x;
    const int c = threadIdx.x;
    const int wave = c / KN_WAVE;
    if (c < PF_M * PF_DSUB) {
        sq[c] = a.queries[q * a.d + c];
    }
    __syncthreads();
    {
        const int cc = c & (PF_KSUB - 1), m0 = (c / PF_KSUB) * (PF_M / 2);
#pragma unroll
        for (int j = 0; j < PF_M / 2; j++) {
            const int m = m0 + j;
            const float4 y = cb_m[m * PF_KSUB + cc];
            const float4 x = *reinterpret_cast<const float4*>(sq + m * PF_DSUB);
            float t = ip_step(0.f, x.x, y.x);
            t = ip_step(t, x.y, y.y);
            t = ip_step(t, x.z, y.z);
            t = ip_step(t, x.w, y.w);
            lut[m * PF_KSUB + cc] = IS_L2 ? fmul_x(-2.0f, t) : t;
        }
    }
    __syncthreads();
    {
#pragma unroll
        for (int j = 0; j < PF_M / PS_WAVES; j++) {
            const int m = wave * (PF_M / PS_WAVES) + j;
            float h = -INFINITY, l = INFINITY;
#pragma unroll
            for (int e = 0; e < PF_KSUB / KN_WAVE; e++) {
                const float v = lut[m * PF_KSUB + lane_id() + e * KN_WAVE];
                const bool fin = fabsf(v) < INFINITY;
                h = fmaxf(h, fin ? v : INFINITY);
                l = fminf(l, fin ? v : -INFINITY);
            }
#pragma unroll
            for (int dlt = KN_WAVE / 2; dlt > 0; dlt >>= 1) {
                h = fmaxf(h, __shfl_xor(h, dlt, KN_WAVE));
                l = fminf(l, __shfl_xor(l, dlt, KN_WAVE));
            }
            if (lane_id() == 0) {
                const float mu = 0.5f * h + 0.5f * l;
                s_mu[m] = mu;
                s_a[m] = fmaxf(fabsf(h), fabsf(l));
                s_r[m] = h - l;
                if (qmu != nullptr) {
                    qmu[q * PF_M + m] = mu;
                }
            }
        }
    }
    __syncthreads();
    if (c == 0) {
        float A = 0.f, R = 0.f, musum = 0.f, gmax = 0.f;
#pragma unroll 4
        for (int m = 0; m < PF_M; m++) {
            musum += s_mu[m];
            A += s_a[m];
            R = fmaxf(R, s_r[m]);
            gmax = fmaxf(gmax, s_a[m]);
        }
        s_A = A;
        float sc = 1.0f, eps = INFINITY;
        if (A < INFINITY) {
            if (gmax > 0.f) {
                int e = 0;
                (void)frexpf(gmax, &e);
                int p2 = 15 - e;
                p2 = p2 > 126 ? 126 : (p2 < -126 ? -126 : p2);
                sc = ldexpf(1.0f, p2);
            }
            const float isc = 1.0f / sc;
            eps = PF_UH * A * 1.001f + 9.5367431640625e-7f * isc + 128.0f * PF_U * (pabs_max + A);
        }
        qs[q * 4 + 0] = sc;
        qs[q * 4 + 1] = 1.0f / sc;
        qs[q * 4 + 2] = eps;
        qs[q * 4 + 3] = A;
        if (qis != nullptr) {
            qis[q * 4 + 0] = R;
            qis[q * 4 + 1] = musum;
            qis[q * 4 + 2] = INFINITY;
            qis[q * 4 + 3] = A;
            if (R > 0.f && R < INFINITY) {
                atomicMax(gl, __float_as_uint(R));
            }
        }
    }
    __syncthreads();
    const float A = s_A;
    int cum = 0;
    for (int slot = 0; slot < a.nslot && cum < smin && cum < scap; slot++) {
        const int64_t key = keys[q * a.nslot + slot];
        const int64_t len = (key >= 0 && key < nlist) ? a.list_len[key] : 0;
        if (len <= 0) {
            continue;
        }
        const int off = cum;
        const int rows = (int)min(len, (int64_t)(scap - cum));
        cum += rows;
        const float dis0 = a.coarse_dis[q * a.nslot + slot];
        const int64_t row_off = a.list_row_off[key];
        const float* ps = a.pq_psum + a.pq_sblk_off_r[key] * 16;
        const float slack0 = 128.0f * PF_U * (pabs_max + A) + 64.0f * PF_U * fabsf(dis0);
        for (int pos0 = c; pos0 < rows; pos0 += PS_ROWS * PS_THREADS) {
            uint4 c0[PS_ROWS], c1[PS_ROWS];
            float psv[PS_ROWS];
#pragma unroll
            for (int u = 0; u < PS_ROWS; u++) {
                const int pos = min(pos0 + u * PS_THREADS, rows - 1);
                const uint4* cp = reinterpret_cast<const uint4*>(a.pq_codes + (row_off + pos) * PF_M);
                c0[u] = cp[0];
                c1[u] = cp[1];
                psv[u] = IS_L2 ? ps[pos] : 0.f;
            }
#pragma unroll
            for (int u = 0; u < PS_ROWS; u++) {
                const int pos = pos0 + u * PS_THREADS;
                const uint32_t w[8] = {c0[u].x, c0[u].y, c0[u].z, c0[u].w, c1[u].x, c1[u].y, c1[u].z, c1[u].w};
                float acc = 0.f;
#pragma unroll
                for (int m = 0; m < PF_M; m++) {
                    acc += lut[m * PF_KSUB + ((w[m >> 2] >> (8 * (m & 3))) & 0xffu)];
                }
                float val = IS_L2 ? (dis0 + psv[u]) + acc : dis0 + acc;
                const float slack = slack0 + 64.0f * PF_U * fabsf(val);
                val = IS_L2 ? val + slack : val - slack;
                if (!(slack < INFINITY) || val != val) {
                    val = worst_dist<IS_L2>();
                }
                if (pos < rows) {
                    if (a.bitset != nullptr && bitset_filtered(a.bitset, a.bitset_nbits, a.ids[row_off + pos])) {
                        val = worst_dist<IS_L2>();
                    }
                    a.dump[q * a.dump_stride + off + pos] = val;
                }
            }
        }
    }
    if (c == 0) {
        n_row[q] = cum;
    }
    if (gthr_out == nullptr) {
        return;
    }
    __syncthreads();
    constexpr int PER = PF_SAMPLE / PS_THREADS;
    uint32_t key[PER];
    uint32_t mn = 0xffffffffu, mx = 0u;
#pragma unroll
    for (int u = 0; u < PER; u++) {
        const int i = c + u * PS_THREADS;
        key[u] = i < cum ? dist_key<IS_L2>(a.dump[q * a.dump_stride + i]) : 0xffffffffu;
        mn = min(mn, key[u]);
        mx = i < cum ? max(mx, key[u]) : mx;
    }
    constexpr int NSTEP = 18;
    __shared__ int s_step[NSTEP][3];
    __shared__ uint32_t s_mn[PS_WAVES], s_mx[PS_WAVES];
    __shared__ uint32_t s_tmin[PS_THREADS];
    __shared__ uint32_t s_cand[PS_CAND];
    __shared__ uint32_t s_bound, s_kth;
    __shared__ int s_ncand;
    s_tmin[c] = mn;
#pragma unroll
    for (int dlt = KN_WAVE / 2; dlt > 0; dlt >>= 1) {
        mn = min(mn, (uint32_t)__shfl_xor((int)mn, dlt, KN_WAVE));
        mx = max(mx, (uint32_t)__shfl_xor((int)mx, dlt, KN_WAVE));
    }
    if (lane_id() == 0) {
        s_mn[wave] = mn;
        s_mx[wave] = mx;
    }
    if (c < NSTEP * 3) {
        (&s_step[0][0])[c] = 0;
    }
    if (c == 0) {
        s_ncand = 0;
    }
    __syncthreads();
    uint32_t lo = s_mn[0], hi = s_mx[0];
    for (int w = 1; w < PS_WAVES; w++) {
        lo = min(lo, s_mn[w]);
        hi = max(hi, s_mx[w]);
    }
    const uint32_t best = lo;
    bool fast = ksel <= PS_THREADS && cum >= ksel && lo < hi;
    if (fast) {
        if (wave == 0) {
            uint32_t v[PS_THREADS / KN_WAVE];
#pragma unroll
            for (int u = 0; u < PS_THREADS / KN_WAVE; u++) {
                v[u] = s_tmin[lane_id() + u * KN_WAVE];
            }
            const uint32_t b = ps_wave_select(v, ksel, lo, hi);
            if (lane_id() == 0) {
                s_bound = b;
            }
        }
        __syncthreads();
        const uint32_t bound = s_bound;
#pragma unroll
        for (int u = 0; u < PER; u++) {
            if (key[u] <= bound) {
                const int at = atomicAdd(&s_ncand, 1);
                if (at < PS_CAND) {
                    s_cand[at] = key[u];
                }
            }
        }
        __syncthreads();
        const int nc = s_ncand;
        if (nc <= PS_CAND) {
            if (wave == 0) {
                uint32_t v[PS_CAND / KN_WAVE];
#pragma unroll
                for (int u = 0; u < PS_CAND / KN_WAVE; u++) {
                    const int i = lane_id() + u * KN_WAVE;
                    v[u] = i < nc ? s_cand[i] : 0xffffffffu;
                }
                const uint32_t kk = ps_wave_select(v, ksel, lo, bound);
                if (lane_id() == 0) {
                    s_kth = kk;
                }
            }
            __syncthreads();
            lo = s_kth;
            hi = lo;
        } else {
            hi = bound;
            fast = false;
        }
    }
    for (int it = 0; it < NSTEP && lo < hi; it++) {
        const uint32_t span = hi - lo;
        const uint32_t q1 = lo + (span >> 2), q2 = lo + (span >> 1), q3 = lo + (span >> 2) + (span >> 1);
        int c1 = 0, c2 = 0, c3 = 0;
#pragma unroll
        for (int u = 0; u < PER; u++) {
            c1 += key[u] <= q1 ? 1 : 0;
            c2 += key[u] <= q2 ? 1 : 0;
            c3 += key[u] <= q3 ? 1 : 0;
        }
#pragma unroll
        for (int dlt = KN_WAVE / 2; dlt > 0; dlt >>= 1) {
            c1 += __shfl_xor(c1, dlt, KN_WAVE);
            c2 += __shfl_xor(c2, dlt, KN_WAVE);
            c3 += __shfl_xor(c3, dlt, KN_WAVE);
        }
        if (lane_id() == 0) {
            if (c1) atomicAdd(&s_step[it][0], c1);
            if (c2) atomicAdd(&s_step[it][1], c2);
            if (c3) atomicAdd(&s_step[it][2], c3);
        }
        __syncthreads();
        const int t1 = s_step[it][0], t2 = s_step[it][1], t3 = s_step[it][2];
        if (t1 >= ksel) {
            hi = q1;
        } else if (t2 >= ksel) {
            lo = q1 + 1;
            hi = q2;
        } else if (t3 >= ksel) {
            lo = q2 + 1;
            hi = q3;
        } else {
            lo = q3 + 1;
        }
    }
    if (c == 0) {
        const float kth = cum >= ksel ? dist_key_inv<IS_L2>(lo) : worst_dist<IS_L2>();
        gthr_out[q] = kth;
        if (gmeta_out != nullptr) {
            uint32_t glo = 0, shift = KN_HIST_OFF;
            if (kth != worst_dist<IS_L2>() && kth == kth) {
                glo = best;
                const uint32_t range = dist_key<IS_L2>(kth) - glo;
                shift = 0;
                while ((range >> shift) >= (uint32_t)(KN_HIST_BINS - 1)) {
                    shift++;
                }
            }
            gmeta_out[q] = make_uint2(glo, shift);
        }
    }
}

hipError_t launch_pq_sample(const MScanArgs& a, const int64_t* keys, const float4* cb_m, int64_t nlist, int smin,
                            int scap, float pabs_max, bool is_l2, int32_t* n_row, float* qs, float* qis, float* qmu,
                            hipStream_t s, float* gthr_out, uint2* gmeta_out, int ksel) {
    if (a.nq <= 0) {
        return hipSuccess;
    }
    if (a.dump == nullptr || scap < 1 || scap > PF_SAMPLE || a.dump_stride < scap) {
        return hipErrorInvalidValue;
    }
    uint32_t* gl = nullptr;
    if (qis != nullptr) {
        hipError_t e = hipMemsetAsync(qis + a.nq * 4, 0, 4 * sizeof(float), s);
        if (e != hipSuccess) {
            return e;
        }
        gl = reinterpret_cast<uint32_t*>(qis + a.nq * 4);
    }
    if (is_l2) {
        hipLaunchKernelGGL(pq_sample_kernel<true>, dim3((unsigned)a.nq), dim3(PS_THREADS), 0, s, a, keys, cb_m, nlist, smin,
                           scap, pabs_max, n_row, qs, qis, qmu, gl, gthr_out, gmeta_out, ksel);
    } else {
        hipLaunchKernelGGL(pq_sample_kernel<false>, dim3((unsigned)a.nq), dim3(PS_THREADS), 0, s, a, keys, cb_m, nlist, smin,
                           scap, pabs_max, n_row, qs, qis, qmu, gl, gthr_out, gmeta_out, ksel);
    }
    return hipGetLastError();
}

__global__ void pqi_prepare_kernel(MScanArgs a, int64_t nrec) {
    const int64_t r = (int64_t)blockIdx.x * blockDim.x + threadIdx.x;
    if (r < 8 * 16) {
        a.pq_ctr[r] = 0;
    }
    if (r >= nrec || r >= *a.nunits_dev) {
        return;
    }
    P16Rec rec{};
    const KnItem it = a.units[r];
    const int npair = it.npair < PI_Q ? it.npair : PI_Q;
    rec.list = it.list;
    rec.npair = npair;
    rec.len = a.list_len[it.list];
    rec.sblk0 = a.pq_sblk_off_r[it.list];
    rec.row_off = a.list_row_off[it.list];
    for (int j = 0; j < PI_Q; j++) {
        const KnPair p = a.pairs[it.pair0 + (j < npair ? j : npair - 1)];
        rec.q[j] = p.q;
        rec.slot[j] = p.slot;
        rec.dis0[j] = a.coarse_dis[(int64_t)p.q * a.nslot + p.slot];
    }
    a.pq_recs16[r] = rec;
}

constexpr int PI_STAGE_CAP = PF_STAGE_CAP / 2;
constexpr int PI_PC_OFF = 576;
constexpr int PI_PC_STRIDE = 384;
static_assert(PI_PC_OFF + 2 * PI_PC_STRIDE <= PF_CTL_BYTES, "control block layout");

template <bool IS_L2>
__device__ __forceinline__ void pqi_emit_raw(const MScanArgs& a, const float* pcp, const int* pqsp, const int (&x)[4],
                                             float ps, int64_t pos, int qb, float s0, float inv0, int64_t row_off) {
    const int negp = IS_L2 ? (int)ceilf(-ps * inv0) : 0;
#pragma unroll
    for (int r = 0; r < 4; r++) {
        if (x[r] <= negp) {
            const int j = qb + r;
            const int T = __float_as_int(pcp[j * 4 + 3]);
            const int y = IS_L2 ? x[r] + T : -(x[r] + T);
            const float f = (float)y;
            const float v = __fmaf_rn(f, s0, IS_L2 ? ps : 0.f);
            const float th = pcp[j * 4];
            if (IS_L2 ? (v <= th) : (v >= th)) {
                const float pcs = pcp[j * 4 + 2];
                const float pess = IS_L2 ? __fmaf_rn(f, s0, pcs + ps) : __fmaf_rn(f, s0, pcs);
                ms_emit<IS_L2>(a, pqsp[j * 2], pqsp[j * 2 + 1], row_off, pos, pess);
            }
        }
    }
}

struct PiFlush {
    int has;
    int32_t q, slot, n;
    float pess;
    uint2 mt;
    uint32_t pos;
};

template <bool IS_L2>
__device__ __forceinline__ void pqi_flush_issue(const MScanArgs& a, unsigned char* smem, int pp, int64_t row_off, float s0,
                                                float inv0, int wave, int lane, PiFlush& fl) {
    static_assert(PI_STAGE_CAP <= PF_THREADS, "one parked record per thread");
    fl.has = 0;
    const int* cnt = reinterpret_cast<const int*>(smem + PF_LUT_BYTES + PF_CTL_BYTES + PF_STAGE_CAP * 16);
    const int n = min(cnt[pp], PI_STAGE_CAP);
    const int i = wave + PF_WAVES * lane;
    if (i >= n) {
        return;
    }
    const float* pcp = reinterpret_cast<const float*>(smem + PF_LUT_BYTES + PI_PC_OFF + pp * PI_PC_STRIDE);
    const int* pqsp = reinterpret_cast<const int*>(pcp + 64);
    const uint4 r0 = *reinterpret_cast<const uint4*>(smem + PF_LUT_BYTES + PF_CTL_BYTES + i * 32);
    const uint4 r1 = *reinterpret_cast<const uint4*>(smem + PF_LUT_BYTES + PF_CTL_BYTES + i * 32 + 16);
    const int x[4] = {(int)r0.x, (int)r0.y, (int)r0.z, (int)r0.w};
    const float ps = __uint_as_float(r1.x);
    const int qb = (int)r1.z;
    fl.pos = r1.y;
    const int negp = IS_L2 ? (int)ceilf(-ps * inv0) : 0;
    if (a.bitset != nullptr && bitset_filtered(a.bitset, a.bitset_nbits, a.ids[row_off + (int64_t)fl.pos])) {
        return;
    }
#pragma unroll
    for (int r = 0; r < 4; r++) {
        if (x[r] <= negp) {
            const int j = qb + r;
            const int T = __float_as_int(pcp[j * 4 + 3]);
            const int y = IS_L2 ? x[r] + T : -(x[r] + T);
            const float f = (float)y;
            const float v = __fmaf_rn(f, s0, IS_L2 ? ps : 0.f);
            const float th = pcp[j * 4];
            if (IS_L2 ? (v <= th) : (v >= th)) {
                const float pcs = pcp[j * 4 + 2];
                const float pess = IS_L2 ? __fmaf_rn(f, s0, pcs + ps) : __fmaf_rn(f, s0, pcs);
                const int32_t q = pqsp[j * 2], slot = pqsp[j * 2 + 1];
                if (!fl.has) {
                    fl.has = 1;
                    fl.q = q;
                    fl.slot = slot;
                    fl.pess = pess;
                    fl.n = atomicAdd(a.cand_cnt + q, 1);
                    fl.mt = a.ghist != nullptr ? a.gmeta[q] : make_uint2(0u, KN_HIST_OFF);
                } else {
                    MScanArgs b = a;
                    b.bitset = nullptr;
                    ms_emit<IS_L2>(b, q, slot, row_off, (int64_t)fl.pos, pess);
                }
            }
        }
    }
}

template <bool IS_L2>
__device__ __forceinline__ void pqi_flush_complete(const MScanArgs& a, const PiFlush& fl) {
    if (!fl.has) {
        return;
    }
    const int32_t q = fl.q;
    if (fl.n < a.cap) {
        a.cand[(int64_t)q * a.cap + fl.n] = ((int64_t)fl.slot << 32) | (int64_t)fl.pos;
        if (a.cand_pess != nullptr) {
            a.cand_pess[(int64_t)q * a.cap + fl.n] = fl.pess;
        }
    } else {
        a.overflow[q] = 1;
        a.overflow[a.nq] = 1;
    }
    if (fl.mt.y != KN_HIST_OFF) {
        atomicAdd(a.ghist + (int64_t)q * KN_HIST_BINS + hist_bin(dist_key<IS_L2>(fl.pess), fl.mt.x, fl.mt.y), 1u);
    }
}

template <bool IS_L2>
__global__ __launch_bounds__(PF_THREADS) void pqi_kernel(MScanArgs a) {
#ifdef KNHIP_PHASE_TIMERS
    unsigned long long tacc[8] = {0, 0, 0, 0, 0, 0, 0, 0};
    unsigned long long tlast = __builtin_amdgcn_s_memtime();
#endif
    extern __shared__ __align__(16) unsigned char smem[];
    constexpr int REC_WORDS = (int)(sizeof(P16Rec) / 4);
    static_assert(REC_WORDS == 64, "mailbox slots of 64 words, one lane per word");
    static_assert(offsetof(P16Rec, npair) == 4 && offsetof(P16Rec, q) == 8 && offsetof(P16Rec, slot) == 72 &&
                  offsetof(P16Rec, dis0) == 136 && offsetof(P16Rec, len) == 200 && offsetof(P16Rec, sblk0) == 208 &&
                  offsetof(P16Rec, row_off) == 216, "P16Rec layout");
    int* ctl = reinterpret_cast<int*>(smem + PF_LUT_BYTES);
    static_assert(8 * 4 + 2 * REC_WORDS * 4 <= PI_PC_OFF, "control block layout");
    const float s0 = pf_sgpr_f(a.pq_qis[(int64_t)a.nq * 4 + 1]);
    const float inv0 = pf_sgpr_f(a.pq_qis[(int64_t)a.nq * 4 + 2]);
// ... 454 lines not shown
```

Measured before the change: 1.573 million.

## Fuse decode-form query prep and guard prediction into the PQ sample kernel

Folds the int8/decode-form query preparation (fp16 query and error record) and the poor-query guard prediction counters into pq_sample_kernel. This removes the separate pqd_query_prep and pqf_predict launches and their extra passes over the sample dump. It also hoists the guard-cache decision ahead of the sample pass and moves hipFuncSetAttribute for the pqd kernels to one-time index prep. The cost is more shared memory and extra work in the sample kernel. The fused prediction uses its own band-count logic, which may differ from the old predict kernel.

```diff
diff --git a/knowhere_amd/csrc/kernels.h b/knowhere_amd/csrc/kernels.h
--- a/knowhere_amd/csrc/kernels.h
+++ b/knowhere_amd/csrc/kernels.h
@@ -293,14 +293,24 @@
                                const int64_t* list_sblk_off, int64_t nlist, uint4* out, hipStream_t s);
 hipError_t launch_pqi_query_table(const float* queries, const float4* cb_m, int d, int64_t nq, bool is_l2, float pabs_max,
                                   void* qi, float* qis, float* qmu, bool stats_done, hipStream_t s);
+struct PqSampleFuse {
+    void* qh16 = nullptr;
+    float* qd = nullptr;
+    const float* pqd_cst = nullptr;
+    int32_t* poor = nullptr;
+    const float* qs2 = nullptr;
+    int cap = 0;
+};
 hipError_t launch_pq_sample(const MScanArgs& a, const int64_t* keys, const float4* cb_m, int64_t nlist, int smin,
                             int scap, float pabs_max, bool is_l2, int32_t* n_row, float* qs, float* qis, float* qmu,
-                            hipStream_t s, float* gthr_out = nullptr, uint2* gmeta_out = nullptr, int ksel = 0);
+                            hipStream_t s, float* gthr_out = nullptr, uint2* gmeta_out = nullptr, int ksel = 0,
+                            const PqSampleFuse* fuse = nullptr);
 hipError_t launch_pqi(const MScanArgs& a, bool is_l2, int64_t units_bound, hipStream_t s);
 
 constexpr int PD_QT = 128;
 size_t pqd_smem();
 bool pqd_supports(int M, int d);
+hipError_t launch_pqd_prepare_device();
 hipError_t launch_pqd_index_prep(const float4* cb, const float* centroids, int64_t ncent, void* cb16, float* st,
                                  uint32_t* scratch, const float* psum, int64_t npsum, float* psum_s, hipStream_t s);
 hipError_t launch_pqd_query_prep(const float* queries, const float4* cb, const float* cst, int64_t nq, bool is_l2,
diff --git a/knowhere_amd/csrc/knhip_api.hip b/knowhere_amd/csrc/knhip_api.hip
--- a/knowhere_amd/csrc/knhip_api.hip
+++ b/knowhere_amd/csrc/knhip_api.hip
@@ -431,6 +431,7 @@
                                   idx->pqd_cb16.p, idx->pqd_st.as<float>(),
                                   reinterpret_cast<uint32_t*>(idx->pqd_st.as<float>() + 8), idx->psum.as<float>(), npsum,
                                   idx->psum_s.as<float>(), nullptr));
+    HIP_TRY(launch_pqd_prepare_device());
     HIP_TRY(hipDeviceSynchronize());
     idx->pqd_ready = true;
     return KNHIP_OK;
@@ -1734,10 +1735,10 @@
         case KNHIP_STAGE_LUT:
             return "pq_query_table_kernel";
         case KNHIP_STAGE_SCAN_RANK0:
-            return kind == KNHIP_IVF_PQ ? "pq_sample_kernel | pq_scan_v2_kernel<DUMP>+row_select_kernel"
+            return kind == KNHIP_IVF_PQ ? "pq_sample_kernel (+ decode-form query records, guard counters) | pq_scan_v2_kernel<DUMP>+row_select_kernel"
                                         : "mscan_flat_kernel<DUMP> | mscan_sq8_kernel<DUMP> +row_select_kernel+ms_tau_kernel";
         case KNHIP_STAGE_TABLES:
-            return "pqi_query_table_kernel | pqf_query_table_kernel +pqf_predict_kernel";
+            return "pqi_query_table_kernel | pqf_query_table_kernel | (KNHIP_PQ_PREPASS=split, int8 form) pqd_query_prep_kernel+pqf_predict_kernel";
         case KNHIP_STAGE_SCAN:
             return kind == KNHIP_IVF_PQ    ? "pqi_kernel | pqf_kernel | pq_scan_q4_kernel | pq_scan_kernel | pq_scan_any_kernel"
                    : kind == KNHIP_IVF_SQ8 ? "mscan_sq8_kernel | sq_scan_kernel"
diff --git a/knowhere_amd/csrc/knhip_api_search.hip b/knowhere_amd/csrc/knhip_api_search.hip
--- a/knowhere_amd/csrc/knhip_api_search.hip
+++ b/knowhere_amd/csrc/knhip_api_search.hip
@@ -514,8 +514,21 @@
     return KNHIP_OK;
 }
 
+struct GuardPlan {
+    bool want_dec = false;
+    int form2 = 2;
+    bool want2 = false;
+    bool guard = false;
+    bool cached = false;
+    bool sync_now = false;
+    bool predict = false;
+    int form = 1;
+    bool fuse_prep = false;
+    bool fuse_predict = false;
+};
+
 int ms_sample_pass(const knhip_index* idx, Workspace* ws, const SearchPlan& plan, const Batch& b, const EnvSearch& env,
-                   const WorkTable& wt, hipStream_t s, MScanArgs& m) {
+                   const WorkTable& wt, const GuardPlan& g, hipStream_t s, MScanArgs& m) {
     const int kind = idx->desc.kind, d = idx->d, k = b.k;
     const bool is_l2 = idx->is_l2;
     const int64_t nq = b.nq, nlist = idx->nlist, sample = mscan_sample_rows();
@@ -558,9 +571,19 @@
             scap = std::max(64, std::min((int)sample, env.pq_sample_rows));
         }
         const bool i8 = plan.pq_want_i8;
+        PqSampleFuse fz;
+        if (g.fuse_prep) {
+            fz.qh16 = ws->ms_qh16.p;
+            fz.qd = ws->ms_qd.as<float>();
+            fz.pqd_cst = idx->pqd_st.as<float>();
+        }
+        if (g.fuse_predict && (g.sync_now || g.predict)) {
+            fz.poor = ws->ms_cand_cnt.as<int32_t>() + 2 * nq + 1;
+            fz.cap = plan.ms_cap;
+        }
         HIP_TRY(launch_pq_sample(ds, b.keys, idx->cb.as<float4>(), nlist, std::max(1024, 8 * k), scap, idx->pabs_max, is_l2,
                                  ws->ms_nrow.as<int32_t>(), ws->ms_qs.as<float>(), i8 ? ws->ms_qis.as<float>() : nullptr,
-                                 i8 ? ws->ms_qmu.as<float>() : nullptr, s, ws->gthr.as<float>(), ws->gmeta.as<uint2>(), k));
+                                 i8 ? ws->ms_qmu.as<float>() : nullptr, s, ws->gthr.as<float>(), ws->gmeta.as<uint2>(), k, &fz));
         return KNHIP_OK;
     }
     HIP_TRY(launch_ms_units(wt.list_count, wt.list_pair_off, nlist, plan.ms_qt0, ws->ms_unit_off.as<int64_t>(),
@@ -628,89 +651,97 @@
     return KNHIP_OK;
 }
 
+int pq_decide(const knhip_index* idx, const GuardPlan& g, const int32_t* poor_h, int64_t n) {
+    if (g.want2 && (idx->pqf_form == g.form2 || (int64_t)poor_h[1] * 4 <= n)) {
+        return g.form2;
+    }
+    return (int64_t)poor_h[0] * 4 > n ? 0 : 1;
+}
+
+GuardPlan pq_guard_plan(const knhip_index* idx, const SearchPlan& plan, const Batch& b, const EnvSearch& env) {
+    GuardPlan g;
+    g.want_dec = pqd_supports(idx->desc.pq_m, idx->d) && (idx->pqf_form == 0 || idx->pqf_form == 3);
+    g.want2 = plan.pq_want_i8 || g.want_dec;
+    g.form2 = g.want_dec ? 3 : 2;
+    g.form = g.want2 ? g.form2 : 1;
+    g.guard = idx->pqf_guard;
+    g.fuse_prep = g.want_dec && !env.pq_prepass_split;
+    g.fuse_predict = !env.pq_prepass_split && (g.want_dec || !plan.pq_want_i8);
+    if (!g.guard) {
+        return g;
+    }
+    g.sync_now = true;
+    std::lock_guard<std::mutex> lk(idx->mu);
+    g.cached = idx->guard_cache.size() < 64 || idx->guard_cache.count({b.k, b.nprobe}) != 0;
+    if (g.cached) {
+        knhip_index::GuardEntry& e = idx->guard_cache[{b.k, b.nprobe}];
+        if (e.pending && hipEventQuery(e.ev) == hipSuccess) {
+            e.pending = false;
+            e.form = pq_decide(idx, g, e.h_poor, e.pending_nq);
+        }
+        e.age++;
+        if (e.form > 0 && !env.guard_sync && (e.age & 63) != 0) {
+            g.sync_now = false;
+            g.form = e.form;
+            if (!e.pending && !e.claimed && (e.age & 3) == 0) {
+                g.predict = true;
+                e.claimed = true;
+            }
+        }
+    }
+    return g;
+}
+
 int pq_choose_form(const knhip_index* idx, Workspace* ws, const SearchPlan& plan, const Batch& b, const EnvSearch& env,
-                   hipStream_t s, MScanArgs& m, PqForm* f) {
+                   const GuardPlan& g, hipStream_t s, MScanArgs& m, PqForm* f) {
     const int64_t nq = b.nq, sample = mscan_sample_rows();
     const int k = b.k, nprobe = b.nprobe;
     const bool is_l2 = idx->is_l2;
-    const bool want_dec = pqd_supports(idx->desc.pq_m, idx->d) && (idx->pqf_form == 0 || idx->pqf_form == 3);
     if (plan.pq_want_i8) {
         HIP_TRY(launch_pqi_query_table(b.q, idx->cb.as<float4>(), idx->d, nq, is_l2, idx->pabs_max, ws->ms_qi.p,
                                        ws->ms_qis.as<float>(), ws->ms_qmu.as<float>(), true, s));
     }
-    if (want_dec) {
-        if (int rc = ensure_pqd(idx)) return rc;
-        HIP_TRY(ws->ms_qh16.reserve((size_t)nq * 128 * 2));
-        HIP_TRY(ws->ms_qd.reserve((size_t)nq * 4 * sizeof(float)));
+    if (g.want_dec && !g.fuse_prep) {
         HIP_TRY(launch_pqd_query_prep(b.q, idx->cb.as<float4>(), idx->pqd_st.as<float>(), nq, is_l2, idx->pabs_max,
                                       ws->ms_qh16.p, ws->ms_qd.as<float>(), s));
     }
-    const bool want2 = plan.pq_want_i8 || want_dec;
-    const int form2 = want_dec ? 3 : 2;
-    const float* qs2 = want_dec ? ws->ms_qd.as<float>() : plan.pq_want_i8 ? ws->ms_qis.as<float>() : nullptr;
-    auto decide = [&](const int32_t* poor_h, int64_t n) -> int {
-        if (want2 && (idx->pqf_form == form2 || (int64_t)poor_h[1] * 4 <= n)) {
-            return form2;
-        }
-        return (int64_t)poor_h[0] * 4 > n ? 0 : 1;
-    };
-    int form = want2 ? form2 : 1;
-    if (idx->pqf_guard) {
+    int form = g.form;
+    if (g.sync_now || g.predict) {
+        const float* qs2 = g.want_dec ? ws->ms_qd.as<float>() : plan.pq_want_i8 ? ws->ms_qis.as<float>() : nullptr;
         int32_t* poor = ws->ms_cand_cnt.as<int32_t>() + 2 * nq + 1;
-        bool predicted = false;
-        auto predict = [&]() -> hipError_t {
-            if (predicted) {
-                return hipSuccess;
+        if (!g.fuse_predict) {
+            HIP_TRY(launch_pqf_predict(ws->dump.as<float>(), sample, ws->ms_nrow.as<int32_t>(), ws->gthr.as<float>(),
+                                       ws->ms_qs.as<float>(), qs2, b.keys, nprobe, idx->nlist, idx->d_list_len.as<int64_t>(), nq,
+                                       plan.ms_cap, k, is_l2, poor, s));
+        }
+        if (g.predict) {
+            std::lock_guard<std::mutex> lk(idx->mu);
+            knhip_index::GuardEntry& e = idx->guard_cache[{k, nprobe}];
+            e.claimed = false;
+            if (e.h_poor == nullptr) {
+                HIP_TRY(hipHostMalloc(reinterpret_cast<void**>(&e.h_poor), 2 * sizeof(int32_t)));
+                HIP_TRY(hipEventCreateWithFlags(&e.ev, hipEventDisableTiming));
             }
-            predicted = true;
-            return launch_pqf_predict(ws->dump.as<float>(), sample, ws->ms_nrow.as<int32_t>(), ws->gthr.as<float>(),
-                                      ws->ms_qs.as<float>(), qs2, b.keys, nprobe, idx->nlist, idx->d_list_len.as<int64_t>(), nq,
-                                      plan.ms_cap, k, is_l2, poor, s);
-        };
-        bool sync_now = true;
-        std::unique_lock<std::mutex> lk(idx->mu);
-        const bool cached = idx->guard_cache.size() < 64 || idx->guard_cache.count({k, nprobe}) != 0;
-        if (cached) {
-            knhip_index::GuardEntry& e = idx->guard_cache[{k, nprobe}];
-            if (e.pending && hipEventQuery(e.ev) == hipSuccess) {
-                e.pending = false;
-                e.form = decide(e.h_poor, e.pending_nq);
-            }
-            e.age++;
-            if (e.form > 0 && !env.guard_sync && (e.age & 63) != 0) {
-                sync_now = false;
-                form = e.form;
-                if (!e.pending && (e.age & 3) == 0) {
-                    HIP_TRY(predict());
-                    if (e.h_poor == nullptr) {
-                        HIP_TRY(hipHostMalloc(reinterpret_cast<void**>(&e.h_poor), 2 * sizeof(int32_t)));
-                        HIP_TRY(hipEventCreateWithFlags(&e.ev, hipEventDisableTiming));
-                    }
-                    HIP_TRY(hipMemcpyAsync(e.h_poor, poor, 2 * sizeof(int32_t), hipMemcpyDeviceToHost, s));
-                    HIP_TRY(hipEventRecord(e.ev, s));
-                    e.pending = true;
-                    e.pending_nq = nq;
-                }
-            }
-        }
-        lk.unlock();
-        if (sync_now) {
-            HIP_TRY(predict());
+            HIP_TRY(hipMemcpyAsync(e.h_poor, poor, 2 * sizeof(int32_t), hipMemcpyDeviceToHost, s));
+            HIP_TRY(hipEventRecord(e.ev, s));
+            e.pending = true;
+            e.pending_nq = nq;
+        } else {
             int32_t h_poor[2] = {0, 0};
             HIP_TRY(hipMemcpyAsync(h_poor, poor, 2 * sizeof(int32_t), hipMemcpyDeviceToHost, s));
             HIP_TRY(hipStreamSynchronize(s));
-            form = decide(h_poor, nq);
-            if (cached) {
-                lk.lock();
+            form = pq_decide(idx, g, h_poor, nq);
+            if (g.cached) {
+                std::lock_guard<std::mutex> lk(idx->mu);
                 knhip_index::GuardEntry& e = idx->guard_cache[{k, nprobe}];
                 if (!e.pending) {
                     e.form = form;
                 }
             }
         }
-        if (form == 0) {
-            return KNHIP_PQF_ABANDONED;
-        }
+    }
+    if (form == 0) {
+        return KNHIP_PQF_ABANDONED;
     }
     f->form = form;
     return pq_bind_form(idx, ws, plan, b, env, s, m, f);
@@ -809,13 +840,23 @@
     if (int rc = ms_common_args(idx, ws, plan, b, wt, s, m)) return rc;
     SideJoin sj{ws, s};
     WorkTable wside;
+    const bool pq = idx->desc.kind == KNHIP_IVF_PQ;
+    GuardPlan g;
+    if (pq) {
+        g = pq_guard_plan(idx, plan, b, env);
+        if (g.want_dec) {
+            if (int rc = ensure_pqd(idx)) return rc;
+            HIP_TRY(ws->ms_qh16.reserve((size_t)b.nq * 128 * 2));
+            HIP_TRY(ws->ms_qd.reserve((size_t)b.nq * 4 * sizeof(float)));
+        }
+    }
     if (int rc = ms_fork_group(idx, ws, plan, b, env, wt, s, &sj, &wside)) return rc;
-    if (int rc = ms_sample_pass(idx, ws, plan, b, env, wt, s, m)) return rc;
+    if (int rc = ms_sample_pass(idx, ws, plan, b, env, wt, g, s, m)) return rc;
     f->qt = plan.ms_qt;
     {
         StageTimer t(idx, s, KNHIP_STAGE_TABLES);
-        if (idx->desc.kind == KNHIP_IVF_PQ) {
-            if (int rc = pq_choose_form(idx, ws, plan, b, env, s, m, f)) return rc;
+        if (pq) {
+            if (int rc = pq_choose_form(idx, ws, plan, b, env, g, s, m, f)) return rc;
         }
     }
     if (int rc = ms_group_units(idx, ws, plan, b, *f, wside, &sj, s, m)) return rc;
diff --git a/knowhere_amd/csrc/knhip_env.h b/knowhere_amd/csrc/knhip_env.h
--- a/knowhere_amd/csrc/knhip_env.h
+++ b/knowhere_amd/csrc/knhip_env.h
@@ -29,6 +29,7 @@
     int pq_sample_rows;
     bool no_side_stream;
     bool guard_sync;
+    bool pq_prepass_split;
     bool range_no_waves;
     bool ties_canonical;
     bool ties_trace;
@@ -87,6 +88,7 @@
     e.pq_sample_rows = b ? std::max(1, std::atoi(b)) : 0;
     e.no_side_stream = std::getenv("KNHIP_NO_SIDE_STREAM") != nullptr;
     e.guard_sync = std::getenv("KNHIP_PQF_GUARD_SYNC") != nullptr;
+    e.pq_prepass_split = env_is(std::getenv("KNHIP_PQ_PREPASS"), "split");
     e.range_no_waves = std::getenv("KNHIP_RANGE_NO_WAVES") != nullptr;
     const char* t = std::getenv("KNHIP_TIES");
     e.ties_canonical = t && (t[0] == 'c' || t[0] == 'C' || t[0] == '0');
diff --git a/knowhere_amd/csrc/knhip_internal.h b/knowhere_amd/csrc/knhip_internal.h
--- a/knowhere_amd/csrc/knhip_internal.h
+++ b/knowhere_amd/csrc/knhip_internal.h
@@ -254,6 +254,7 @@
         int32_t* h_poor = nullptr;
         hipEvent_t ev = nullptr;
         bool pending = false;
+        bool claimed = false;
         int64_t pending_nq = 0;
         int age = 0;
     };
diff --git a/knowhere_amd/csrc/ms_common.h b/knowhere_amd/csrc/ms_common.h
--- a/knowhere_amd/csrc/ms_common.h
+++ b/knowhere_amd/csrc/ms_common.h
@@ -127,4 +127,62 @@
     return __ballot(v);
 }
 
+#ifndef PD_EXP
+#define PD_EXP 0
+#endif
+constexpr int PD_M = 32;
+constexpr int PD_KSUB = 256;
+constexpr int PD_D = 128;
+constexpr float PD_U = 5.9604645e-8f;
+constexpr float PD_UH = 4.8828125e-4f;
+constexpr float PD_A = 6.103515625e-5f;
+
+__device__ __forceinline__ float pqd_abs_entry(const float* q4, const float4& e) {
+    return fabsf(q4[0]) * fabsf(e.x) + fabsf(q4[1]) * fabsf(e.y) + fabsf(q4[2]) * fabsf(e.z) + fabsf(q4[3]) * fabsf(e.w);
 }
+__device__ __forceinline__ void pqd_abs_max(float v, uint32_t* s_max) {
+#pragma unroll
+    for (int dlt = KN_WAVE / 2; dlt > 0; dlt >>= 1) {
+        v = fmaxf(v, __shfl_xor(v, dlt, KN_WAVE));
+    }
+    if (lane_id() == 0) {
+        atomicMax(s_max, __float_as_uint(v));
+    }
+}
+template <bool IS_L2>
+__device__ __forceinline__ float pqd_query_record(const float* s_q, const uint32_t* s_max, const float* __restrict__ cst,
+                                                  float pabs_max, float* __restrict__ rec) {
+    const float inv_y = cst[1], ysum = cst[3], sc_q = cst[4], inv_q = cst[5], inv_sc = cst[7];
+    float B = 0.f, q1 = 0.f;
+    bool fits = true;
+    for (int m = 0; m < PD_M; m++) {
+        B += __uint_as_float(s_max[m]);
+    }
+    for (int i = 0; i < PD_D; i++) {
+        q1 += fabsf(s_q[i]);
+        fits = fits && fabsf(s_q[i]) * sc_q < 65504.0f;
+    }
+    B *= 1.0001f;
+    q1 *= 1.0001f;
+    float eps = INFINITY;
+    if (fits && B < INFINITY) {
+        const float F = IS_L2 ? 2.0f : 1.0f;
+        const float e_prod = (2.0f * PD_UH + PD_UH * PD_UH) * B;
+        const float e_sub = PD_A * (1.0f + PD_UH) * (ysum * inv_q + q1 * inv_y) + 128.0f * PD_A * PD_A * inv_sc;
+        const float e_acc = 136.0f * PD_U * ((1.0f + 3.0f * PD_UH) * B + 0.5f * pabs_max);
+        eps = (F * (e_prod + e_sub + e_acc) + 128.0f * PD_U * (pabs_max + F * B)) * 1.001f;
+#if defined(PD_EXP) && (PD_EXP & 32)
+        eps *= 16.0f;
+#endif
+#if defined(PD_EXP) && (PD_EXP & 64)
+        eps *= 0.25f;
+#endif
+    }
+    rec[0] = q1;
+    rec[1] = B;
+    rec[2] = eps;
+    rec[3] = 2.0f * B;
+    return eps;
+}
+
+}
diff --git a/knowhere_amd/csrc/pq_decode.hip b/knowhere_amd/csrc/pq_decode.hip
--- a/knowhere_amd/csrc/pq_decode.hip
+++ b/knowhere_amd/csrc/pq_decode.hip
@@ -9,12 +9,6 @@
 
 namespace knhip {
 
-#ifndef PD_EXP
-#define PD_EXP 0
-#endif
-constexpr int PD_M = 32;
-constexpr int PD_KSUB = 256;
-constexpr int PD_D = 128;
 constexpr int PD_WAVES = 4;
 constexpr int PD_THREADS = PD_WAVES * KN_WAVE;
 constexpr int PD_CB_BYTES = PD_M * PD_KSUB * 8;
@@ -32,9 +26,6 @@
 constexpr int PD_OFF_W = PD_CB_BYTES;
 constexpr int PD_SMEM = PD_OFF_W + PD_WAVES * PD_W_BYTES;
 static_assert(PD_SMEM <= 160 * 1024, "LDS of one workgroup");
-constexpr float PD_U = 5.9604645e-8f;
-constexpr float PD_UH = 4.8828125e-4f;
-constexpr float PD_A = 6.103515625e-5f;
 
 #ifdef KNHIP_PHASE_TIMERS
 #define PD_T(i)                                                         \
@@ -185,53 +176,16 @@
         s_max[c] = 0u;
     }
     __syncthreads();
-    const float inv_y = cst[1], ysum = cst[3], sc_q = cst[4], inv_q = cst[5], inv_sc = cst[7];
+    const float sc_q = cst[4];
     if (c < PD_D) {
         qh16[q * PD_D + c] = (_Float16)(s_q[c] * sc_q);
     }
     for (int m = 0; m < PD_M; m++) {
-        const float4 e = cb[m * PD_KSUB + c];
-        float v = fabsf(s_q[4 * m]) * fabsf(e.x) + fabsf(s_q[4 * m + 1]) * fabsf(e.y) + fabsf(s_q[4 * m + 2]) * fabsf(e.z) +
-                  fabsf(s_q[4 * m + 3]) * fabsf(e.w);
-#pragma unroll
-        for (int dlt = KN_WAVE / 2; dlt > 0; dlt >>= 1) {
-            v = fmaxf(v, __shfl_xor(v, dlt, KN_WAVE));
-        }
-        if (lane_id() == 0) {
-            atomicMax(&s_max[m], __float_as_uint(v));
-        }
+        pqd_abs_max(pqd_abs_entry(s_q + 4 * m, cb[m * PD_KSUB + c]), &s_max[m]);
     }
     __syncthreads();
     if (c == 0) {
-        float B = 0.f, q1 = 0.f;
-        bool fits = true;
-        for (int m = 0; m < PD_M; m++) {
-            B += __uint_as_float(s_max[m]);
-        }
-        for (int i = 0; i < PD_D; i++) {
-            q1 += fabsf(s_q[i]);
-            fits = fits && fabsf(s_q[i]) * sc_q < 65504.0f;
-        }
-        B *= 1.0001f;
-        q1 *= 1.0001f;
-        float eps = INFINITY;
-        if (fits && B < INFINITY) {
-            const float F = IS_L2 ? 2.0f : 1.0f;
-            const float e_prod = (2.0f * PD_UH + PD_UH * PD_UH) * B;
-            const float e_sub = PD_A * (1.0f + PD_UH) * (ysum * inv_q + q1 * inv_y) + 128.0f * PD_A * PD_A * inv_sc;
-            const float e_acc = 136.0f * PD_U * ((1.0f + 3.0f * PD_UH) * B + 0.5f * pabs_max);
-            eps = (F * (e_prod + e_sub + e_acc) + 128.0f * PD_U * (pabs_max + F * B)) * 1.001f;
-#if defined(PD_EXP) && (PD_EXP & 32)
-            eps *= 16.0f;
-#endif
-#if defined(PD_EXP) && (PD_EXP & 64)
-            eps *= 0.25f;
-#endif
-        }
-        qd[q * 4 + 0] = q1;
-        qd[q * 4 + 1] = B;
-        qd[q * 4 + 2] = eps;
-        qd[q * 4 + 3] = 2.0f * B;
+        (void)pqd_query_record<IS_L2>(s_q, s_max, cst, pabs_max, qd + q * 4);
     }
 }
 
@@ -969,6 +923,18 @@
 #endif
 }
 
+hipError_t launch_pqd_prepare_device() {
+    const void* kerns[4] = {reinterpret_cast<const void*>(pqd_kernel<true, true>), reinterpret_cast<const void*>(pqd_kernel<false, true>),
+                            reinterpret_cast<const void*>(pqd_kernel<true, false>), reinterpret_cast<const void*>(pqd_kernel<false, false>)};
+    for (const void* kern : kerns) {
+        hipError_t e = hipFuncSetAttribute(kern, hipFuncAttributeMaxDynamicSharedMemorySize, (int)PD_SMEM);
+        if (e != hipSuccess) {
+            return e;
+        }
+    }
+    return hipSuccess;
+}
+
 hipError_t launch_pqd(const MScanArgs& a, bool is_l2, int64_t units_bound, hipStream_t s) {
     if (units_bound <= 0) {
         return hipSuccess;
@@ -985,13 +951,8 @@
     }
     auto kern = a.unit_loop ? (is_l2 ? pqd_kernel<true, true> : pqd_kernel<false, true>)
                             : (is_l2 ? pqd_kernel<true, false> : pqd_kernel<false, false>);
-    hipError_t e = hipFuncSetAttribute(reinterpret_cast<const void*>(kern), hipFuncAttributeMaxDynamicSharedMemorySize,
-                                       (int)PD_SMEM);
-    if (e != hipSuccess) {
-        return e;
-    }
     if (!a.unit_loop) {
-        e = hipMemsetAsync(a.pq_ctr, 0, 8 * 16 * sizeof(int32_t), s);
+        hipError_t e = hipMemsetAsync(a.pq_ctr, 0, 8 * 16 * sizeof(int32_t), s);
         if (e != hipSuccess) {
             return e;
         }
diff --git a/knowhere_amd/csrc/pq_filter.hip b/knowhere_amd/csrc/pq_filter.hip
--- a/knowhere_amd/csrc/pq_filter.hip
+++ b/knowhere_amd/csrc/pq_filter.hip
@@ -1015,16 +1015,26 @@
                                                             float* __restrict__ qs, float* __restrict__ qis,
                                                             float* __restrict__ qmu, uint32_t* __restrict__ gl,
                                                             float* __restrict__ gthr_out, uint2* __restrict__ gmeta_out,
-                                                            int ksel) {
+                                                            int ksel, PqSampleFuse fz) {
     __shared__ float lut[PF_M * PF_KSUB];
     __shared__ float sq[PF_M * PF_DSUB];
     __shared__ float s_mu[PF_M], s_a[PF_M], s_r[PF_M];
     __shared__ float s_A;
+    __shared__ uint32_t s_bmax[PF_M];
+    __shared__ float s_eps[2];
+    __shared__ int s_band[3];
     const int64_t q = blockIdx.x;
     const int c = threadIdx.x;
     const int wave = c / KN_WAVE;
+    const bool dec = fz.qd != nullptr;
     if (c < PF_M * PF_DSUB) {
         sq[c] = a.queries[q * a.d + c];
+    }
+    if (c < PF_M) {
+        s_bmax[c] = 0u;
+    }
+    if (c < 3) {
+        s_band[c] = 0;
     }
     __syncthreads();
     {
@@ -1039,6 +1049,12 @@
             t = ip_step(t, x.z, y.z);
             t = ip_step(t, x.w, y.w);
             lut[m * PF_KSUB + cc] = IS_L2 ? fmul_x(-2.0f, t) : t;
+            if (dec) {
+                pqd_abs_max(pqd_abs_entry(sq + m * PF_DSUB, y), &s_bmax[m]);
+            }
+        }
+        if (dec && c < PD_D) {
+            static_cast<_Float16*>(fz.qh16)[q * PD_D + c] = (_Float16)(sq[c] * fz.pqd_cst[4]);
         }
     }
     __syncthreads();
@@ -1097,6 +1113,7 @@
         qs[q * 4 + 1] = 1.0f / sc;
         qs[q * 4 + 2] = eps;
         qs[q * 4 + 3] = A;
+        s_eps[0] = eps;
         if (qis != nullptr) {
             qis[q * 4 + 0] = R;
             qis[q * 4 + 1] = musum;
@@ -1106,6 +1123,9 @@
                 atomicMax(gl, __float_as_uint(R));
             }
         }
+    }
+    if (dec && c == KN_WAVE) {
+        s_eps[1] = pqd_query_record<IS_L2>(sq, s_bmax, fz.pqd_cst, IS_L2 ? pabs_max : 0.f, fz.qd + q * 4);
     }
     __syncthreads();
     const float A = s_A;
@@ -1287,6 +1307,49 @@
             lo = q3 + 1;
         }
     }
+    if (fz.poor != nullptr) {
+        const float tau = cum >= ksel ? dist_key_inv<IS_L2>(lo) : worst_dist<IS_L2>();
+        if (tau != worst_dist<IS_L2>() && cum > 0) {
+            const bool two = dec || fz.qs2 != nullptr;
+            const float eps1 = s_eps[0] + 64.0f * PF_U * fabsf(tau);
+            const float eps2 = two ? (dec ? s_eps[1] : fz.qs2[q * 4 + 2]) + 64.0f * PF_U * fabsf(tau) : 0.f;
+            const uint32_t kt = lo;
+            const uint32_t kl1 = dist_key<IS_L2>(IS_L2 ? tau + 2.0f * eps1 : tau - 2.0f * eps1);
+            const uint32_t kl2 = dist_key<IS_L2>(IS_L2 ? tau + 2.0f * eps2 : tau - 2.0f * eps2);
+            int c1 = 0, c2 = 0, rows = 0;
+#pragma unroll
+            for (int u = 0; u < PER; u++) {
+                const bool in = c + u * PS_THREADS < cum && key[u] > kt;
+                c1 += (in && key[u] <= kl1) ? 1 : 0;
+                c2 += (in && key[u] <= kl2) ? 1 : 0;
+            }
+            for (int sl = c; sl < a.nslot; sl += PS_THREADS) {
+                const int64_t lk = keys[q * a.nslot + sl];
+                rows += (lk >= 0 && lk < nlist) ? (int)a.list_len[lk] : 0;
+            }
+#pragma unroll
+            for (int dlt = KN_WAVE / 2; dlt > 0; dlt >>= 1) {
+                c1 += __shfl_xor(c1, dlt, KN_WAVE);
+                c2 += __shfl_xor(c2, dlt, KN_WAVE);
+                rows += __shfl_xor(rows, dlt, KN_WAVE);
+            }
+            if (lane_id() == 0) {
+                if (c1) atomicAdd(&s_band[0], c1);
+                if (c2) atomicAdd(&s_band[1], c2);
+                if (rows) atomicAdd(&s_band[2], rows);
+            }
+            __syncthreads();
+            if (c == 0) {
+                const float rw = (float)s_band[2], n = (float)cum;
+                if ((float)ksel + (float)s_band[0] / n * rw > 0.5f * (float)fz.cap) {
+                    atomicAdd(fz.poor, 1);
+                }
+                if (two && (float)ksel + (float)s_band[1] / n * rw > 0.5f * (float)fz.cap) {
+                    atomicAdd(fz.poor + 1, 1);
+                }
+            }
+        }
+    }
     if (c == 0) {
         const float kth = cum >= ksel ? dist_key_inv<IS_L2>(lo) : worst_dist<IS_L2>();
         gthr_out[q] = kth;
@@ -1307,12 +1370,23 @@
 
 hipError_t launch_pq_sample(const MScanArgs& a, const int64_t* keys, const float4* cb_m, int64_t nlist, int smin,
                             int scap, float pabs_max, bool is_l2, int32_t* n_row, float* qs, float* qis, float* qmu,
-                            hipStream_t s, float* gthr_out, uint2* gmeta_out, int ksel) {
+                            hipStream_t s, float* gthr_out, uint2* gmeta_out, int ksel, const PqSampleFuse* fuse) {
     if (a.nq <= 0) {
         return hipSuccess;
     }
     if (a.dump == nullptr || scap < 1 || scap > PF_SAMPLE || a.dump_stride < scap) {
         return hipErrorInvalidValue;
+    }
+    const PqSampleFuse fz = fuse != nullptr ? *fuse : PqSampleFuse{};
+    if ((fz.qd != nullptr) != (fz.qh16 != nullptr) || (fz.qd != nullptr && fz.pqd_cst == nullptr) ||
+        (fz.poor != nullptr && gthr_out == nullptr)) {
+        return hipErrorInvalidValue;
+    }
+    if (fz.poor != nullptr) {
+        hipError_t e = hipMemsetAsync(fz.poor, 0, 2 * sizeof(int32_t), s);
+        if (e != hipSuccess) {
+            return e;
+        }
     }
     uint32_t* gl = nullptr;
     if (qis != nullptr) {
@@ -1324,10 +1398,10 @@
     }
     if (is_l2) {
         hipLaunchKernelGGL(pq_sample_kernel<true>, dim3((unsigned)a.nq), dim3(PS_THREADS), 0, s, a, keys, cb_m, nlist, smin,
-                           scap, pabs_max, n_row, qs, qis, qmu, gl, gthr_out, gmeta_out, ksel);
+                           scap, pabs_max, n_row, qs, qis, qmu, gl, gthr_out, gmeta_out, ksel, fz);
     } else {
         hipLaunchKernelGGL(pq_sample_kernel<false>, dim3((unsigned)a.nq), dim3(PS_THREADS), 0, s, a, keys, cb_m, nlist, smin,
-                           scap, pabs_max, n_row, qs, qis, qmu, gl, gthr_out, gmeta_out, ksel);
+                           scap, pabs_max, n_row, qs, qis, qmu, gl, gthr_out, gmeta_out, ksel, fz);
     }
     return hipGetLastError();
 }
```

Measured after the change: 1.570 million. About the same (-0.2%).
